# vitoplantamura/OnnxStream

Hardware: NVIDIA H100
Metric: SD1.5 UNet 512x512 bs=1 denoise steps/s (one UNet Model::run per step) (higher is better)
Workload: dtype f16

## Files before the change

### include/onnxstream_b200_kernels.h

```cpp
#ifndef ONNXSTREAM_B200_KERNELS_H
#define ONNXSTREAM_B200_KERNELS_H

#include <stddef.h>
#include <stdint.h>

#ifdef __cplusplus
extern "C" {
#endif

enum { OSB_NONE = 0, OSB_U8 = 1, OSB_F16 = 2, OSB_F32 = 3, OSB_I64 = 4 };

#define OSB_MAX_DIMS 6

int osb_convert(const void* src, int src_dtype, void* dst, int dst_dtype, size_t n, float scale, int zero_point, void* stream);

enum { OSB_UN_SIGMOID = 0, OSB_UN_SILU, OSB_UN_ERF, OSB_UN_SQRT, OSB_UN_SIN, OSB_UN_COS, OSB_UN_POW, OSB_UN_NEG,
       OSB_UN_GELU_ERF, OSB_UN_COPY, OSB_UN_MULC, OSB_UN_ADDC, OSB_UN_RECIP_SQRT };
int osb_unary(int op, const void* x, void* y, int dtype, size_t n, float alpha, void* stream);

enum { OSB_BIN_ADD = 0, OSB_BIN_SUB, OSB_BIN_MUL, OSB_BIN_DIV, OSB_BIN_MUL_GELU, OSB_BIN_MUL_SIGMOID, OSB_BIN_SILU_MUL  };
int osb_binary(int op, const void* a, const int64_t* a_strides, const void* b, const int64_t* b_strides,
               void* out, const int64_t* out_shape, int ndim, int dtype, void* stream);

int osb_bf16x3_expand_cols(const void* in_f32, void* out_bf16, int64_t rows, int64_t L, int64_t ld_in, int b_side, void* stream);
int osb_bf16x3_expand_rows(const void* in_f32, void* out_bf16, int64_t K, int64_t N, int b_side, void* stream);
int osb_tc_gemm_f32x_ok(int64_t M, int64_t N, int64_t K);
int osb_tc_conv_f32x_ok(int64_t H, int64_t W, int64_t Cin, int64_t Cout, int kh, int kw, int stride, int64_t Ho, int64_t Wo);
int osb_tc_gemm_f32x(const void* A6, const void* B6, void* C_f32, const void* bias_f32, const void* residual_f32, int64_t M, int64_t N, int64_t K6, int b_transposed, void* stream);
int osb_tc_conv_f32x(const void* x6, const void* w6, const void* bias_f32, const void* residual_f32, void* y_f32, int64_t H, int64_t W, int64_t Cin6, int64_t Cout,
                     int kh, int kw, int stride, int pad_top, int pad_left, int64_t Ho, int64_t Wo, void* stream);
int osb_concat2(const void* a, const void* b, void* out, int64_t outer, int64_t a_bytes, int64_t b_bytes, void* stream);
int osb_strided_copy(const void* in, void* out, int elem_size, int ndim, const int64_t* shape,
                     const int64_t* in_stride, const int64_t* in_div, int64_t in_offset,
                     const int64_t* out_stride, int64_t out_offset, void* stream);

int osb_transpose2d(const void* in, void* out, int elem_size, int64_t batch, int64_t rows, int64_t cols, void* stream);

int osb_softmax(const void* x, void* y, int dtype, int64_t rows, int64_t cols, void* stream);

int osb_softmax_scaled(const void* x, void* y, int dtype, int64_t rows, int64_t cols, float scale, const void* mask, int64_t mask_rows, void* stream);
int osb_softmax_scaled_ld(const void* x, void* y, int dtype, int64_t rows, int64_t cols, int64_t ld, float scale, const void* mask, int64_t mask_rows, void* stream);

int osb_instance_norm(const void* x, void* y, int dtype, int64_t channels, int64_t n_per_channel,
                      const void* scale, const void* bias, float eps, void* stream);

int osb_group_norm(const void* x, void* y, int dtype, int nhwc, int64_t C, int64_t HW, int groups,
                   const void* gamma, const void* beta, float eps, int fuse_silu, void* stats, void* stream);

int osb_geglu(const void* x, void* y, int dtype, int64_t rows, int64_t inner, void* stream);

int osb_layer_norm(const void* x, void* y, int dtype, int64_t rows, int64_t cols, const void* gamma, const void* beta,
                   float eps, void* stream);

int osb_reduce_mean(const void* x, void* y, int dtype, int64_t rows, int64_t cols, void* stream);

int osb_gather_rows(const void* table, const int64_t* idx, void* out, int64_t n_idx, int64_t table_rows, int64_t row_bytes, void* stream);

int osb_gemm(const void* A, const void* B, void* C, const void* bias, const void* residual,
             int64_t batch, int64_t M, int64_t N, int64_t K,
             int64_t stride_a, int64_t stride_b, int64_t stride_c, int b_transposed, int dtype, int impl, void* stream);

int osb_gemm_grouped(const void* A, const void* const* B, void* const* C, int groups, int64_t M, int64_t N, int64_t K,
                     int b_transposed, int dtype, int impl, void* stream);

int osb_gemm_ld(const void* A, int64_t lda, const void* B, int64_t ldb, void* C, int64_t ldc, const void* bias, const void* residual,
                int64_t batch, int64_t M, int64_t N, int64_t K, int64_t stride_a, int64_t stride_b, int64_t stride_c,
                int b_transposed, int dtype, int impl, void* stream);

int osb_conv2d(const void* x, const void* w, const void* bias, const void* residual, void* y,
               int64_t H, int64_t W, int64_t Cin, int64_t Cout, int kh, int kw, int stride, int pad_top, int pad_left,
               int64_t Ho, int64_t Wo, int dtype, int impl, void* stream);
int osb_conv2d_ex(const void* x, const void* w, const void* bias, const void* bias2, const void* residual, void* y, int64_t H, int64_t W, int64_t Cin, int64_t Cout,
                  int kh, int kw, int stride, int pad_top, int pad_left, int64_t Ho, int64_t Wo, int dtype, int impl, void* stream,
                  void* gn_stats, int gn_groups, int* gn_done);
int osb_conv2d_fusable(const void* x, const void* w, const void* y, int64_t H, int64_t W, int64_t Cin, int64_t Cout, int kh, int kw, int stride, int dtype, int impl);
int osb_rms_norm(const void* x, int xd, const void* w, int wd, void* y, int yd, int64_t rows, int64_t cols, float eps, void* stream);
int osb_rope(const void* x, const void* cs, const void* sn, void* y, int dtype, int64_t rows, int64_t D, int64_t table_rows, void* stream);
int osb_gemv_w8(const void* A, const void* Wq, void* C, const void* bias, const void* residual, int64_t M, int64_t N, int64_t K, float wscale, int wzp, int dtype, void* stream);
int osb_gemv_grouped(const void* A, const void* const* B, void* const* C, const int64_t* N, const float* wscale, const int* wzp, int groups,
                     int64_t M, int64_t K, int wdtype, int dtype, void* stream);
int osb_qu8_tc_gemm_ok(int64_t M, int64_t N, int64_t K, const void* A, const void* B, const void* C);
int osb_qu8_tc_conv_ok(int64_t Cin, int64_t Cout, int64_t Ho, int64_t Wo, int kh, int kw, int stride, const void* x, const void* w, const void* y);
int osb_rowsum_u8(const void* x, void* out, int64_t rows, int64_t cols, void* stream);
int osb_colsum_u8(const void* w, void* out, int64_t K, int64_t N, void* stream);
int osb_pad_sum_u8(const void* x, void* xp, void* psum, int64_t H, int64_t W, int64_t C, int64_t Hp, int64_t Wp, int pad_top, int pad_left, int zx, void* stream);
int osb_qu8_tc_gemm(const void* A, const void* B, void* C, const void* bias, const void* rsum, const void* csum, int64_t M, int64_t N, int64_t K, int bt,
                    int zx, float sx, int zw, float sw, int zy, float sy, void* stream);
int osb_qu8_tc_conv(const void* xp, const void* psum, const void* w, const void* bias, const void* csum, void* y, int64_t Hp, int64_t Wp, int64_t Cin, int64_t Cout,
                    int kh, int kw, int stride, int64_t Ho, int64_t Wo, int zx, float sx, int zw, float sw, int zy, float sy, void* stream);
int osb_binary_qu8(int op, const void* a, const int64_t* as, float sa, int za, const void* b, const int64_t* bs, float sb, int zb,
                   void* out, float so, int zo, const int64_t* shape, int ndim, void* stream);
int osb_softmax_qu8(const void* x, void* y, int64_t rows, int64_t cols, float in_scale, float out_scale, int out_zp, void* stream);
int osb_percentiles(const void* x, int dtype, size_t n, int threads, float from_left, float from_right, void* out3, void* stream);
float osb_percentile_key_to_float(unsigned key, int dtype);
int osb_channel_add_stats(const void* x, const void* addv, void* y, int dtype, int64_t C, int64_t HW, int groups, void* stats, void* stream);
int osb_group_norm_apply(const void* x, void* y, int dtype, int64_t C, int64_t HW, int groups, const void* gamma, const void* beta, float eps, int fuse_silu,
                         const void* stats, void* clear_stats, void* stream);

int osb_attention(const void* q, const void* k, const void* v, const void* mask, void* out,
                  int64_t heads, int64_t Tq, int64_t Tk, int64_t d, int64_t dv, float scale, int k_transposed,
                  int64_t kv_group, int dtype, void* stream);

int osb_flash_attention_ok(int64_t T, int64_t Tk, int64_t d, int dtype);
int osb_flash_attention(const void* q, int64_t ldq, const void* k, int64_t ldk, const void* v, int64_t ldv, void* out, int64_t ldo,
                        int64_t heads, int64_t T, int64_t Tk, int64_t d, float scale, void* stream);

int osb_flash_attention_f32x_ok(int64_t T, int64_t Tk, int64_t d, int dtype);
int osb_flash_attention_f32x(const void* q, int64_t ldq, const void* k, int64_t ldk, const void* v, int64_t ldv, void* out, int64_t ldo,
                             int64_t heads, int64_t T, int64_t Tk, int64_t d, float scale, void* planes, void* stream);

int osb_flash_attention_wide_ok(int64_t T, int64_t Tk, int64_t d, int dtype);
int osb_flash_attention_wide(const void* q, const void* k, const void* v, void* out, int64_t heads, int64_t T, int64_t Tk, int64_t d,
                             float scale, int k_transposed, int dtype, void* stream);

int osb_flash_attention_wide_f32x_ok(int64_t T, int64_t Tk, int64_t d, int dtype);
int osb_flash_attention_wide_f32x(const void* q, const void* k, const void* v, void* out, int64_t heads, int64_t T, int64_t Tk, int64_t d,
                                  float scale, int k_transposed, void* planes, void* stream);

int osb_sdpa_flash_ok(int64_t Hq, int64_t Hkv, int64_t Tq, int64_t Tk, int64_t d, int64_t dv, int dtype);
int osb_sdpa_flash(const void* q, const void* k, const void* v, const void* mask, void* out,
                   int64_t Hq, int64_t Hkv, int64_t Tq, int64_t Tk, int64_t d, float scale, void* stream);

int osb_gemm_qu8(const uint8_t* A, const uint8_t* B, uint8_t* C, const int32_t* bias, int64_t M, int64_t N, int64_t K,
                 int zx, float sx, int zw, float sw, int zy, float sy, void* stream);
int osb_conv2d_qu8(const uint8_t* x, const uint8_t* w, const int32_t* bias, uint8_t* y,
                   int64_t H, int64_t W, int64_t Cin, int64_t Cout, int kh, int kw, int stride, int pad_top, int pad_left,
                   int64_t Ho, int64_t Wo, int zx, float sx, int zw, float sw, int zy, float sy, void* stream);

int osb_scatter_elems(void* out, const int64_t* pos, const void* updates, int64_t n, int elem_size, void* stream);

int osb_maxpool_nhwc(const void* x, void* y, int dtype, int64_t H, int64_t W, int64_t C, int kh, int kw, int stride, int pad_top,
                     int pad_left, int64_t Ho, int64_t Wo, void* stream);

int osb_fill(void* dst, int dtype, size_t n, float value, void* stream);

int osb_gemm_tc_eligible(int64_t M, int64_t N, int64_t K, int dtype);

void osb_tc_set_pair_mode(int mode);

void osb_tc_profile(int enable);
int osb_tc_profile_read(double* out4);
int osb_tc_profile_dump(char* buf, int cap);

int osb_pdl_enabled(void);
void osb_set_pdl(int enable);

uint64_t osb_launch_count(void);
void osb_launch_count_reset(void);
uint64_t osb_tc_launch_count(void);

#ifdef __cplusplus
}
#endif
#endif
```

### onnxstream_b200/csrc/gemm_wgmma.cu

```cuda

#include "common.cuh"
#include "workspace.h"
#include "tc_ptx.cuh"
#include <cuda.h>
#include <cstdio>
#include <cstdlib>
#include <vector>

namespace {

constexpr int BLOCK_M = 128;
constexpr int BLOCK_N = 128;
constexpr int BLOCK_K = 64;
constexpr int WG_K = 16;
constexpr int STAGES = 6;
constexpr int A_STAGE_BYTES = BLOCK_M * BLOCK_K * 2;
constexpr int B_STAGE_BYTES = BLOCK_N * BLOCK_K * 2;
constexpr int SMEM_BYTES = STAGES * (A_STAGE_BYTES + B_STAGE_BYTES) + 1024  + 256  + 2 * tcptx::GN_MAX_GROUPS * 4;
constexpr int NUM_THREADS = 384;
constexpr int CONSUMER_THREADS = 256;

struct TcParams {
    int M, N, K;
    int batch;
    int m_tiles, n_tiles;
    int b_kmajor;
    int a_swap, b_swap;
    int taps, kw, pad_top, pad_left, Wo, Ho, bw, bh, tiles_x;
    int k_blocks_per_tap;
    int stride;
    int split_k;
    float* ws;
    int groups;
    __half* C1;
    __half* C2;
    __half* C;
    const __half* bias;
    const __half* bias2;
    const __half* residual;
    double* gn_stats;
    int gn_cpg, gn_groups;
    int gn_debug;
    int bf16;
    int f32_out;
    long long stride_c;
    long long ldc;
};

using namespace tcptx;

template <int B_MN_MAJOR, bool BF16>
__device__ __forceinline__ void mma_kblock(float (&acc)[64], uint64_t adesc, uint64_t bdesc)
{
    constexpr uint32_t b_kstep = B_MN_MAJOR ? (WG_K * 128) >> 4 : (WG_K * 2) >> 4;
    wgmma_fence();
#pragma unroll
    for (int k = 0; k < BLOCK_K / WG_K; k++) {
        const uint64_t a = adesc + (uint64_t)(k * ((WG_K * 2) >> 4)), b = bdesc + (uint64_t)(k * b_kstep);
        if (BF16) wgmma_m64n128k16_bf16<B_MN_MAJOR>(acc, a, b, 1u);
        else wgmma_m64n128k16_f16<B_MN_MAJOR>(acc, a, b, 1u);
    }
    wgmma_commit();
}


template <bool EXTRAS, int B_MN_MAJOR, bool BF16, bool PAIR>
__global__ void __launch_bounds__(NUM_THREADS, 1)
tc_gemm_kernel(const __grid_constant__ CUtensorMap map_a, const __grid_constant__ CUtensorMap map_b, const __grid_constant__ CUtensorMap map_b1,
               const __grid_constant__ CUtensorMap map_b2, const TcParams p)
{
    osb_pdl_trigger_entry();
    extern __shared__ uint8_t smem_raw[];
    uint8_t* smem = (uint8_t*)(((uintptr_t)smem_raw + 1023) & ~(uintptr_t)1023);
    uint8_t* smem_a = smem;
    uint8_t* smem_b = smem + STAGES * A_STAGE_BYTES;
    uint64_t* bars = (uint64_t*)(smem + STAGES * (A_STAGE_BYTES + B_STAGE_BYTES));
    uint64_t* full = bars;
    uint64_t* empty = bars + STAGES;
    float* gn_acc = (float*)((uint8_t*)bars + 256);

    const int warp = threadIdx.x >> 5;
    const int lane = threadIdx.x & 31;
    if (EXTRAS && p.gn_stats && threadIdx.x < 2 * GN_MAX_GROUPS) gn_acc[threadIdx.x] = 0.f;

    if (warp == 0 && lane == 0) {
        asm volatile("prefetch.tensormap [%0];" ::"l"(&map_a) : "memory");
        asm volatile("prefetch.tensormap [%0];" ::"l"(&map_b) : "memory");
    }
    constexpr uint32_t EMPTY_ARRIVALS = PAIR ? 2 * (CONSUMER_THREADS / 32) : CONSUMER_THREADS;
    if (warp == 1 && lane == 0) {
        for (int i = 0; i < STAGES; i++) { mbar_init(&full[i], 1); mbar_init(&empty[i], EMPTY_ARRIVALS); }
        asm volatile("fence.mbarrier_init.release.cluster;" ::: "memory");
    }
    if (PAIR) cluster_sync();
    else __syncthreads();
    osb_pdl_wait();

    const uint32_t rank = PAIR ? cluster_ctarank() : 0;
    const int first = PAIR ? (int)cluster_id_x() : (int)blockIdx.x, step = PAIR ? (int)cluster_count_x() : (int)gridDim.x;
    const int m_units = PAIR ? (p.m_tiles + 1) / 2 : p.m_tiles;
    const int tiles_per_batch = m_units * p.n_tiles;
    const int total_tiles = tiles_per_batch * p.batch * p.split_k;
    const int k_blocks_all = p.taps * p.k_blocks_per_tap;
    const int kb_per_split = (k_blocks_all + p.split_k - 1) / p.split_k;

    if (warp == 0) {
        const uint32_t sa0 = smem_u32(smem_a), sb0 = smem_u32(smem_b);
        int stage = 0; uint32_t phase = 0;
        for (int tile = first; tile < total_tiles; tile += step) {
            int sp = tile % p.split_k, t2 = tile / p.split_k;
            int b = t2 / tiles_per_batch, r = t2 % tiles_per_batch;
            int mt = r % m_units, nt = r / m_units;
            if (PAIR) mt = 2 * mt + (int)rank;
            int n0 = nt * BLOCK_N;
            int y0 = 0, x0 = 0, m0 = mt * BLOCK_M;
            if (p.taps > 1 || p.bh > 0) { y0 = (mt / p.tiles_x) * p.bh; x0 = (mt % p.tiles_x) * p.bw; }
            const CUtensorMap* mbp = &map_b;
            if (p.groups > 1) { if (b == 1) mbp = &map_b1; else if (b == 2) mbp = &map_b2; b = 0; }
            int kb_lo = sp * kb_per_split, kb_hi = min(kb_lo + kb_per_split, k_blocks_all);
            int tap = kb_lo / p.k_blocks_per_tap, kcb = kb_lo % p.k_blocks_per_tap;
            int ky = tap / p.kw, kx = tap % p.kw;
            const int ax = x0 * p.stride - p.pad_left, ay = y0 * p.stride - p.pad_top;
            for (int kb = kb_lo; kb < kb_hi; kb++) {
                mbar_wait(&empty[stage], phase ^ 1);
                if (elect_one()) {
                    mbar_expect_tx(&full[stage], A_STAGE_BYTES + B_STAGE_BYTES);
                    const int kc = kcb * BLOCK_K;
                    const uint32_t sa = sa0 + stage * A_STAGE_BYTES;
                    const uint32_t sb = sb0 + stage * B_STAGE_BYTES;
                    if (p.bh > 0) tma_load_3d_s(sa, &map_a, &full[stage], kc, ax + kx, ay + ky);
                    else if (p.a_swap) tma_load_3d_s(sa, &map_a, &full[stage], kc, b, m0);
                    else tma_load_3d_s(sa, &map_a, &full[stage], kc, m0, b);
                    const int kglob = tap * p.K + kc;
                    if (PAIR) {
                        const uint32_t sbh = sb + rank * (B_STAGE_BYTES / 2);
                        const int nh = n0 + 64 * (int)rank;
                        if (p.b_kmajor) {
                            if (p.b_swap) tma_load_3d_mc(sbh, mbp, &full[stage], kglob, b, nh, 0x3);
                            else tma_load_3d_mc(sbh, mbp, &full[stage], kglob, nh, b, 0x3);
                        } else {
                            if (p.b_swap) tma_load_3d_mc(sbh, mbp, &full[stage], nh, b, kglob, 0x3);
                            else tma_load_3d_mc(sbh, mbp, &full[stage], nh, kglob, b, 0x3);
                        }
                    } else if (p.b_kmajor) {
                        if (p.b_swap) tma_load_3d_s(sb, mbp, &full[stage], kglob, b, n0);
                        else tma_load_3d_s(sb, mbp, &full[stage], kglob, n0, b);
                    } else {
                        if (p.b_swap) {
                            tma_load_3d_s(sb, mbp, &full[stage], n0, b, kglob);
                            tma_load_3d_s(sb + B_STAGE_BYTES / 2, mbp, &full[stage], n0 + 64, b, kglob);
                        } else {
                            tma_load_3d_s(sb, mbp, &full[stage], n0, kglob, b);
                            tma_load_3d_s(sb + B_STAGE_BYTES / 2, mbp, &full[stage], n0 + 64, kglob, b);
                        }
                    }
                }
                __syncwarp();
                if (++kcb == p.k_blocks_per_tap) { kcb = 0; tap++; if (++kx == p.kw) { kx = 0; ky++; } }
                if (++stage == STAGES) { stage = 0; phase ^= 1; }
            }
        }
        osb_pdl_trigger_late();
    } else if (warp >= 4) {
        const int wg = (warp >> 2) - 1;
        const int ct = (int)threadIdx.x - (NUM_THREADS - CONSUMER_THREADS);
        const uint64_t adesc0 = make_smem_desc(smem_u32(smem_a) + wg * (BLOCK_M / 2) * 128, 16, 1024);
        const uint64_t bdesc0 = p.b_kmajor ? make_smem_desc(smem_u32(smem_b), 16, 1024) : make_smem_desc(smem_u32(smem_b), B_STAGE_BYTES / 2, 1024);
        const bool partial = p.split_k > 1 || p.f32_out;
        const int r_lo = wg * 64 + (warp & 3) * 16 + (lane >> 2);
        const int cq = 2 * (lane & 3);
        auto release = [&](int s) {
            if (PAIR) {
                __syncwarp();
                if (lane == 0) { mbar_arrive(&empty[s]); mbar_arrive_remote(&empty[s], rank ^ 1u); }
            } else {
                mbar_arrive(&empty[s]);
            }
        };
        int stage = 0; uint32_t phase = 0;
        for (int tile = first; tile < total_tiles; tile += step) {
            int sp = tile % p.split_k, t2 = tile / p.split_k;
            int b = t2 / tiles_per_batch, r = t2 % tiles_per_batch;
            int mt = r % m_units, nt = r / m_units;
            if (PAIR) mt = 2 * mt + (int)rank;
            const int n0 = nt * BLOCK_N;
            const int n_end = min(p.N, n0 + BLOCK_N);
            const int kb_lo = sp * kb_per_split, kb_hi = min(kb_lo + kb_per_split, k_blocks_all);

            float acc[64];
#pragma unroll
            for (int i = 0; i < 64; i++) acc[i] = 0.f;
            int prev = -1;
            for (int kb = kb_lo; kb < kb_hi; kb++) {
                mbar_wait(&full[stage], phase);
                mma_kblock<B_MN_MAJOR, BF16>(acc, adesc0 + (uint64_t)(stage * (A_STAGE_BYTES >> 4)), bdesc0 + (uint64_t)(stage * (B_STAGE_BYTES >> 4)));
                if (prev >= 0) { wgmma_wait<1>(); release(prev); }
                prev = stage;
                if (++stage == STAGES) { stage = 0; phase ^= 1; }
            }
            wgmma_wait<0>();
            release(prev);

            long long out_row[2];
            bool row_ok[2];
#pragma unroll
            for (int h = 0; h < 2; h++) {
                const int row_in_tile = r_lo + 8 * h;
                if (p.bh > 0) {
                    int y = (mt / p.tiles_x) * p.bh + row_in_tile / p.bw, x = (mt % p.tiles_x) * p.bw + row_in_tile % p.bw;
                    row_ok[h] = y < p.Ho && x < p.Wo;
                    out_row[h] = (long long)y * p.Wo + x;
                } else {
                    int m = mt * BLOCK_M + row_in_tile;
                    row_ok[h] = m < p.M;
                    out_row[h] = m;
                }
            }
            __half* cbase = p.C;
            if (p.groups > 1) cbase = b == 0 ? p.C : (b == 1 ? p.C1 : p.C2);
            const bool pair_ok = (p.N & 1) == 0 && (p.ldc & 1) == 0;
#pragma unroll
            for (int j = 0; j < BLOCK_N / 8; j++) {
                if (n0 + 8 * j >= n_end) break;
                const int n = n0 + 8 * j + cq;
                const bool ok0 = n < n_end, ok1 = n + 1 < n_end;
                float s0 = 0.f, s1 = 0.f, q0 = 0.f, q1 = 0.f;
                float add0 = 0.f, add1 = 0.f;
                if (!partial) {
                    if (p.bias) { if (ok0) add0 += __half2float(p.bias[n]); if (ok1) add1 += __half2float(p.bias[n + 1]); }
                }
#pragma unroll
                for (int h = 0; h < 2; h++) {
                    if (!row_ok[h]) continue;
                    float f0 = acc[4 * j + 2 * h], f1 = acc[4 * j + 2 * h + 1];
                    if (partial) {
                        float* wrow = p.ws + (((long long)sp * p.batch + b) * p.M + out_row[h]) * p.N;
                        if (ok1 && pair_ok) *reinterpret_cast<float2*>(wrow + n) = make_float2(f0, f1);
                        else { if (ok0) wrow[n] = f0; if (ok1) wrow[n + 1] = f1; }
                        continue;
                    }
                    const long long off = (long long)b * p.stride_c + out_row[h] * p.ldc;
                    f0 += add0; f1 += add1;
                    if (p.residual) { if (ok0) f0 += __half2float(p.residual[off + n]); if (ok1) f1 += __half2float(p.residual[off + n + 1]); }
                    if (EXTRAS && p.bias2) { if (ok0) f0 += __half2float(p.bias2[n]); if (ok1) f1 += __half2float(p.bias2[n + 1]); }
                    const __half o0 = __float2half_rn(f0), o1 = __float2half_rn(f1);
                    __half* crow = cbase + off;
                    if (ok1 && pair_ok) *reinterpret_cast<__half2*>(crow + n) = __halves2half2(o0, o1);
                    else { if (ok0) crow[n] = o0; if (ok1) crow[n + 1] = o1; }
                    if (EXTRAS) {
                        const float g0 = ok0 ? __half2float(o0) : 0.f, g1 = ok1 ? __half2float(o1) : 0.f;
                        s0 += g0; q0 = fmaf(g0, g0, q0); s1 += g1; q1 = fmaf(g1, g1, q1);
                    }
                }
                if (EXTRAS && p.gn_stats && !partial && !(p.gn_debug & 1)) gn_stats_pair(s0, s1, q0, q1, n, n_end, p.gn_cpg, gn_acc, lane);
            }
            if (EXTRAS && p.gn_stats && !partial && !(p.gn_debug & 2)) {
                asm volatile("bar.sync 1, %0;" ::"n"(CONSUMER_THREADS) : "memory");
                gn_stats_flush(gn_acc, p.gn_stats, p.gn_groups, ct);
            }
        }
    }
    if (PAIR) cluster_sync();
}

__global__ void splitk_reduce_kernel(const float* __restrict__ ws, __half* __restrict__ out, const __half* __restrict__ bias, const __half* __restrict__ bias2,
                                     const __half* __restrict__ residual, long long rows, int N, int splits, double* __restrict__ gn_stats, int gn_cpg, int gn_groups)
{
    osb_pdl_prologue();
    __shared__ float acc[2 * GN_MAX_GROUPS];
    if (gn_stats) { if (threadIdx.x < 2 * GN_MAX_GROUPS) acc[threadIdx.x] = 0.f; __syncthreads(); }
    const long long total4 = rows * N / 4;
    const long long plane4 = total4;
    const float4* w4 = reinterpret_cast<const float4*>(ws);
    for (long long i = blockIdx.x * (long long)blockDim.x + threadIdx.x; i < total4; i += (long long)gridDim.x * blockDim.x) {
        float4 a = w4[i];
        for (int s = 1; s < splits; s++) { float4 t = w4[(long long)s * plane4 + i]; a.x += t.x; a.y += t.y; a.z += t.z; a.w += t.w; }
        long long e = i * 4;
        int n = (int)(e % N);
        if (bias) { a.x += __half2float(bias[n]); a.y += __half2float(bias[n + 1]); a.z += __half2float(bias[n + 2]); a.w += __half2float(bias[n + 3]); }
        if (bias2) { a.x += __half2float(bias2[n]); a.y += __half2float(bias2[n + 1]); a.z += __half2float(bias2[n + 2]); a.w += __half2float(bias2[n + 3]); }
        if (residual) {
            Vec<__half, 4> r = load_vec<__half, 4>(residual + e);
            a.x += __half2float(r.v[0]); a.y += __half2float(r.v[1]); a.z += __half2float(r.v[2]); a.w += __half2float(r.v[3]);
        }
        Vec<__half, 4> o;
        o.v[0] = __float2half_rn(a.x); o.v[1] = __float2half_rn(a.y); o.v[2] = __float2half_rn(a.z); o.v[3] = __float2half_rn(a.w);
        store_vec<__half, 4>(out + e, o);
        if (gn_stats) {
            float x0 = __half2float(o.v[0]), x1 = __half2float(o.v[1]), x2 = __half2float(o.v[2]), x3 = __half2float(o.v[3]);
            const int g = n / gn_cpg;
            atomicAdd(&acc[2 * g], (x0 + x1) + (x2 + x3));
            atomicAdd(&acc[2 * g + 1], fmaf(x0, x0, x1 * x1) + fmaf(x2, x2, x3 * x3));
        }
    }
    if (gn_stats) {
        __syncthreads();
        if (threadIdx.x < 2 * gn_groups) { float v = acc[threadIdx.x]; if (v != 0.f) atomicAdd(&gn_stats[threadIdx.x], (double)v); }
    }
}

__global__ void splitk_reduce_f32_kernel(const float* __restrict__ ws, float* __restrict__ out, const float* __restrict__ bias, const float* __restrict__ residual,
                                         long long rows, int N, int splits)
{
    osb_pdl_prologue();
    const long long total = rows * N;
    for (long long i = blockIdx.x * (long long)blockDim.x + threadIdx.x; i < total; i += (long long)gridDim.x * blockDim.x) {
        float a = ws[i];
        for (int s = 1; s < splits; s++) a += ws[(long long)s * total + i];
        if (bias) a += bias[(int)(i % N)];
        if (residual) a += residual[i];
        out[i] = a;
    }
}

#include "gemm_i8.cuh"

constexpr size_t WS_MAX = OSB_WS_SPLITK_BYTES;

int num_sms();

int choose_split(int tiles, int k_blocks, size_t out_elems, cudaStream_t st, OsbWorkspace** ws_out)
{
    static const int forced = [] { const char* e = getenv("OSB_TC_SPLIT"); return e ? atoi(e) : 0; }();
    *ws_out = nullptr;
    static const int min_kb = [] { const char* e = getenv("OSB_TC_SPLIT_MINKB"); int v = e ? atoi(e) : 0; return v > 0 ? v : 32; }();
    if ((tiles >= 100 && forced <= 0) || k_blocks < 4 || (k_blocks < min_kb && forced <= 0)) return 1;
    int split = forced > 0 ? forced : num_sms() / tiles;
    split = std::min(split, k_blocks / 2);
    while (split > 1 && (size_t)split * out_elems * 4 > WS_MAX) split--;
    if (split <= 1) return 1;
    int kb_per = (k_blocks + split - 1) / split;
    split = (k_blocks + kb_per - 1) / kb_per;
    if (split <= 1) return 1;
    OsbWorkspace* ws = osb_workspace(st, OSB_WS_SPLITK);
    if (!ws) return 1;
    *ws_out = ws;
    return split;
}

bool make_map_rb(CUtensorMap* map, const void* base, uint64_t inner, uint64_t rows, uint64_t batch, uint64_t row_stride_bytes, uint64_t batch_stride_bytes,
                 uint32_t box_inner, uint32_t box_rows, int* swapped)
{
    if (batch > 1 && batch_stride_bytes < row_stride_bytes) {
        *swapped = 1;
        return make_map(map, base, inner, batch, rows, batch_stride_bytes, row_stride_bytes, box_inner, 1, box_rows);
    }
    *swapped = 0;
    return make_map(map, base, inner, rows, batch, row_stride_bytes, batch_stride_bytes, box_inner, box_rows, 1);
}

int num_sms()
{
    static int n = 0;
    if (!n) { int dev = 0; cudaGetDevice(&dev); cudaDeviceGetAttribute(&n, cudaDevAttrMultiProcessorCount, dev); if (n <= 0) n = 132; }
    return n;
}

struct ProfRec { cudaEvent_t a, b; double flops, bytes; int M, N, K, taps, batch, split, conv; };
bool g_prof = false;
std::vector<ProfRec> g_prof_list;

void prof_begin(ProfRec& rec, const TcParams& p, cudaStream_t st)
{
    cudaEventCreate(&rec.a); cudaEventCreate(&rec.b);
    const double kdiv = p.bf16 ? 6.0 : 1.0, es = p.bf16 ? 4.0 : 2.0;
    double M = p.M, N = p.N, Kt = (double)p.K * p.taps / kdiv, B = p.batch;
    rec.flops = 2.0 * M * N * Kt * B;
    double a_bytes = (p.bh > 0 ? M * (p.K / kdiv) : M * Kt) * es * B;
    rec.bytes = a_bytes + N * Kt * es * (p.bh > 0 ? 1.0 : B) + M * N * es * B * (p.residual ? 2.0 : 1.0) + (p.bias ? N * es : 0.0);
    rec.M = p.M; rec.N = p.N; rec.K = p.K; rec.taps = p.taps; rec.batch = p.batch; rec.split = p.split_k; rec.conv = p.bh > 0;
    cudaEventRecord(rec.a, st);
}

using TcKernel = void (*)(CUtensorMap, CUtensorMap, CUtensorMap, CUtensorMap, TcParams);

int launch(const CUtensorMap& ma, const CUtensorMap& mb, const TcParams& p, cudaStream_t st, const CUtensorMap* mb1p = nullptr, const CUtensorMap* mb2p = nullptr,
           bool pair = false)
{
    const CUtensorMap& mb1 = mb1p ? *mb1p : mb;
    const CUtensorMap& mb2 = mb2p ? *mb2p : mb;
    static bool attr_set = false;
    if (!attr_set) {
        TcKernel kernels[] = {
            tc_gemm_kernel<false, 0, false, false>, tc_gemm_kernel<false, 1, false, false>, tc_gemm_kernel<true, 0, false, false>, tc_gemm_kernel<true, 1, false, false>,
            tc_gemm_kernel<false, 0, true, false>, tc_gemm_kernel<false, 1, true, false>,
            tc_gemm_kernel<false, 0, false, true>, tc_gemm_kernel<false, 1, false, true>, tc_gemm_kernel<true, 0, false, true>, tc_gemm_kernel<true, 1, false, true> };
        for (auto k : kernels) {
            cudaError_t e = cudaFuncSetAttribute(k, cudaFuncAttributeMaxDynamicSharedMemorySize, SMEM_BYTES);
            if (e != cudaSuccess) return (int)e;
        }
        attr_set = true;
    }
    const bool extras = p.bias2 != nullptr || p.gn_stats != nullptr;
    TcKernel k;
    if (pair) {
        if (p.bf16 || p.split_k != 1 || p.groups > 1) return (int)cudaErrorInvalidValue;
        k = extras ? (p.b_kmajor ? tc_gemm_kernel<true, 0, false, true> : tc_gemm_kernel<true, 1, false, true>)
                   : (p.b_kmajor ? tc_gemm_kernel<false, 0, false, true> : tc_gemm_kernel<false, 1, false, true>);
    } else if (p.bf16) {
        k = p.b_kmajor ? tc_gemm_kernel<false, 0, true, false> : tc_gemm_kernel<false, 1, true, false>;
    } else if (extras) {
        k = p.b_kmajor ? tc_gemm_kernel<true, 0, false, false> : tc_gemm_kernel<true, 1, false, false>;
    } else {
        k = p.b_kmajor ? tc_gemm_kernel<false, 0, false, false> : tc_gemm_kernel<false, 1, false, false>;
    }
    int grid;
    if (pair) {
        static int max_clusters = 0;
        if (!max_clusters) {
            cudaLaunchConfig_t cfg{};
            cfg.gridDim = dim3(2 * (num_sms() / 2)); cfg.blockDim = dim3(NUM_THREADS); cfg.dynamicSmemBytes = SMEM_BYTES;
            cudaLaunchAttribute attr[1];
            attr[0].id = cudaLaunchAttributeClusterDimension;
            attr[0].val.clusterDim.x = 2; attr[0].val.clusterDim.y = 1; attr[0].val.clusterDim.z = 1;
            cfg.attrs = attr; cfg.numAttrs = 1;
            int n = 0;
            if (cudaOccupancyMaxActiveClusters(&n, k, &cfg) != cudaSuccess || n <= 0) { cudaGetLastError(); n = num_sms() / 2; }
            max_clusters = std::min(n, num_sms() / 2);
        }
        const int units = (p.m_tiles + 1) / 2 * p.n_tiles * p.batch;
        grid = 2 * std::min(units, max_clusters);
    } else {
        grid = std::min(p.m_tiles * p.n_tiles * p.batch * p.split_k, num_sms());
    }
    ProfRec rec{};
    if (g_prof) prof_begin(rec, p, st);
    osb_launch_cluster(k, grid, NUM_THREADS, (size_t)SMEM_BYTES, st, pair ? 2u : 1u, ma, mb, mb1, mb2, p);
    if (p.f32_out) {
        launched(1);
        const long long total = (long long)p.batch * p.M * p.N;
        int rgrid = (int)std::min<long long>((total + 255) / 256, num_sms() * 8);
        osb_launch((splitk_reduce_f32_kernel), rgrid, 256, 0, st, (const float*)p.ws, (float*)p.C, (const float*)p.bias, (const float*)p.residual, (long long)p.batch * p.M, p.N, p.split_k);
        if (g_prof) { cudaEventRecord(rec.b, st); g_prof_list.push_back(rec); }
        return launched(0);
    }
    if (p.split_k > 1) {
        launched(1);
        long long total4 = (long long)p.batch * p.M * p.N / 4;
        int rgrid = (int)std::min<long long>((total4 + 255) / 256, num_sms() * 8);
        osb_launch((splitk_reduce_kernel), rgrid, 256, 0, st, (const float*)p.ws, p.C, p.bias, p.bias2, p.residual, (long long)p.batch * p.M, p.N, p.split_k,
                   p.gn_stats, p.gn_cpg, p.gn_groups);
        if (g_prof) { cudaEventRecord(rec.b, st); g_prof_list.push_back(rec); }
        return launched(0);
    }
    if (g_prof) { cudaEventRecord(rec.b, st); g_prof_list.push_back(rec); }
    return launched(1);
}

int env_int(const char* name)
{
    const char* e = getenv(name);
    return e ? atoi(e) : 0;
}

inline uint32_t next_pow2(uint32_t v) { uint32_t r = 1; while (r < v) r <<= 1; return r; }

int g_pair_mode = -1;
int pair_mode()
{
    if (g_pair_mode < 0) { const char* e = getenv("OSB_TC_PAIR"); g_pair_mode = e ? atoi(e) : 1; }
    return g_pair_mode;
}

bool use_pair(int64_t m_tiles, int64_t N)
{
    return pair_mode() == 2 && m_tiles >= 2 && N % 8 == 0;
}

}

extern "C" void osb_tc_set_pair_mode(int mode) { g_pair_mode = mode; }

extern "C" void osb_tc_profile(int enable)
{
    for (auto& r : g_prof_list) { cudaEventDestroy(r.a); cudaEventDestroy(r.b); }
    g_prof_list.clear();
    g_prof = enable != 0;
}

extern "C" int osb_tc_profile_read(double* out4)
{
    double ms = 0, fl = 0, by = 0;
    for (auto& r : g_prof_list) {
        if (cudaEventSynchronize(r.b) != cudaSuccess) return -1;
        float t = 0.f;
        if (cudaEventElapsedTime(&t, r.a, r.b) != cudaSuccess) return -1;
        ms += t; fl += r.flops; by += r.bytes;
    }
    out4[0] = (double)g_prof_list.size(); out4[1] = ms; out4[2] = fl; out4[3] = by;
    return 0;
}

extern "C" int osb_tc_profile_dump(char* buf, int cap)
{
    int off = 0;
    for (auto& r : g_prof_list) {
        float t = 0.f;
        if (cudaEventSynchronize(r.b) != cudaSuccess || cudaEventElapsedTime(&t, r.a, r.b) != cudaSuccess) return -1;
        int n = snprintf(buf + off, cap - off, "%d %d %d %d %d %d %d %.4f %.3f\n", r.M, r.N, r.K, r.taps, r.batch, r.split, r.conv, t, r.flops * 1e-9);
        if (n < 0 || off + n >= cap) break;
        off += n;
    }
    return off;
}


extern "C" int osb_qu8_tc_gemm_ok(int64_t M, int64_t N, int64_t K, const void* A, const void* B, const void* C)
{
    if (M < 32 || N < 16 || K < 16 || (N % 16) || (K % 16)) return 0;
    if (((uintptr_t)A | (uintptr_t)B | (uintptr_t)C) & 15) return 0;
    static const int off = env_int("OSB_QU8_TC_OFF");
    return get_encode() != nullptr && !off;
}

extern "C" int osb_qu8_tc_conv_ok(int64_t Cin, int64_t Cout, int64_t Ho, int64_t Wo, int kh, int kw, int stride, const void* x, const void* w, const void* y)
{
    if ((Cin % 16) || (Cout % 16) || Ho * Wo < 64 || kh > 7 || kw > 7 || stride < 1 || stride > 2) return 0;
    if (((uintptr_t)x | (uintptr_t)w | (uintptr_t)y) & 15) return 0;
    static const int off = env_int("OSB_QU8_TC_OFF");
    return get_encode() != nullptr && !off;
}

extern "C" int osb_rowsum_u8(const void* x, void* out, int64_t rows, int64_t cols, void* stream)
{
    if (rows * cols == 0) return 0;
    osb_launch((i8k::rowsum_u8_kernel), (unsigned)std::min<int64_t>((rows + 7) / 8, num_sms() * 8), 256, 0, (cudaStream_t)stream, (const uint8_t*)x, (int32_t*)out, (long long)rows, (long long)cols);
    return launched();
}

extern "C" int osb_colsum_u8(const void* w, void* out, int64_t K, int64_t N, void* stream)
{
    if (K * N == 0) return 0;
    cudaStream_t st = (cudaStream_t)stream;
    cudaError_t e = cudaMemsetAsync(out, 0, (size_t)N * 4, st);
    if (e != cudaSuccess) return (int)e;
    const int64_t gx = (N + 255) / 256;
    const int64_t gy = std::max<int64_t>(1, std::min<int64_t>((K + 63) / 64, (num_sms() * 4 + gx - 1) / gx));
    const int64_t k_per = (K + gy - 1) / gy;
    osb_launch((i8k::colsum_u8_kernel), dim3((unsigned)gx, (unsigned)((K + k_per - 1) / k_per)), 256, 0, st, (const uint8_t*)w, (int32_t*)out, (long long)K, (long long)N, (long long)k_per);
    return launched();
}

extern "C" int osb_pad_sum_u8(const void* x, void* xp, void* psum, int64_t H, int64_t W, int64_t C, int64_t Hp, int64_t Wp, int pad_top, int pad_left, int zx, void* stream)
{
    if (Hp * Wp * C == 0) return 0;
    if (C % 16) return (int)cudaErrorInvalidValue;
    osb_launch((i8k::pad_sum_u8_kernel), (unsigned)std::min<int64_t>((Hp * Wp + 7) / 8, num_sms() * 16), 256, 0, (cudaStream_t)stream, (const uint8_t*)x, (uint8_t*)xp, (int32_t*)psum,
               (int)H, (int)W, (int)C, (int)Hp, (int)Wp, pad_top, pad_left, zx);
    return launched();
}

static int launch_i8(const CUtensorMap& ma, const CUtensorMap& mb, const i8k::I8Params& p, cudaStream_t st)
{
    static bool attr_set = false;
    if (!attr_set) {
        cudaError_t e = cudaFuncSetAttribute(i8k::tc_i8_kernel, cudaFuncAttributeMaxDynamicSharedMemorySize, i8k::I8_SMEM);
        if (e != cudaSuccess) return (int)e;
        attr_set = true;
    }
    const int total = p.m_tiles * p.n_tiles;
    osb_launch((i8k::tc_i8_kernel), std::min(total, num_sms()), NUM_THREADS, (size_t)i8k::I8_SMEM, st, ma, mb, p);
    return launched(1);
}

extern "C" int osb_qu8_tc_gemm(const void* A, const void* B, void* C, const void* bias, const void* rsum, const void* csum, int64_t M, int64_t N, int64_t K, int bt,
                               int zx, float sx, int zw, float sw, int zy, float sy, void* stream)
{
    CUtensorMap ma, mb;
    if (!make_map(&ma, A, (uint64_t)K, (uint64_t)M, 1, (uint64_t)K, (uint64_t)M * K, i8k::I8_BLOCK_K, BLOCK_M, 1, 1, CU_TENSOR_MAP_DATA_TYPE_UINT8)) return (int)cudaErrorInvalidValue;
    bool ok = bt ? make_map(&mb, B, (uint64_t)K, (uint64_t)N, 1, (uint64_t)K, (uint64_t)N * K, i8k::I8_BLOCK_K, BLOCK_N, 1, 1, CU_TENSOR_MAP_DATA_TYPE_UINT8)
                 : make_map(&mb, B, (uint64_t)N, (uint64_t)K, 1, (uint64_t)N, (uint64_t)N * K, BLOCK_N, i8k::I8_BLOCK_K, 1, 1, CU_TENSOR_MAP_DATA_TYPE_UINT8);
    if (!ok) return (int)cudaErrorInvalidValue;
    i8k::I8Params p{};
    p.M = (int)M; p.N = (int)N; p.K = (int)K;
    p.m_tiles = (int)((M + BLOCK_M - 1) / BLOCK_M); p.n_tiles = (int)((N + BLOCK_N - 1) / BLOCK_N);
    p.b_kmajor = bt ? 1 : 0;
    p.taps = 1; p.kw = 1; p.bh = 0; p.bw = 0; p.tiles_x = 1; p.stride = 1;
    p.k_blocks_per_tap = (int)((K + i8k::I8_BLOCK_K - 1) / i8k::I8_BLOCK_K);
    p.rsum = (const int32_t*)rsum; p.csum = (const int32_t*)csum; p.bias = (const int32_t*)bias;
    p.zx = zx; p.zw = zw; p.zy = zy; p.kzz = (int)(K * zx * zw); p.requant = sx * sw / sy;
    p.C = (uint8_t*)C; p.ldc = N;
    return launch_i8(ma, mb, p, (cudaStream_t)stream);
}

extern "C" int osb_qu8_tc_conv(const void* xp, const void* psum, const void* w, const void* bias, const void* csum, void* y, int64_t Hp, int64_t Wp, int64_t Cin, int64_t Cout,
                               int kh, int kw, int stride, int64_t Ho, int64_t Wo, int zx, float sx, int zw, float sw, int zy, float sy, void* stream)
{
    const uint32_t bw = std::min<uint32_t>(128, next_pow2((uint32_t)Wo)), bh = 128 / bw;
    CUtensorMap ma, mb;
    const int64_t Ktot = (int64_t)kh * kw * Cin;
    if (!make_map(&ma, xp, (uint64_t)Cin, (uint64_t)Wp, (uint64_t)Hp, (uint64_t)Cin, (uint64_t)Wp * Cin, i8k::I8_BLOCK_K, bw * stride, bh * stride, (uint32_t)stride, CU_TENSOR_MAP_DATA_TYPE_UINT8))
        return (int)cudaErrorInvalidValue;
    if (!make_map(&mb, w, (uint64_t)Ktot, (uint64_t)Cout, 1, (uint64_t)Ktot, (uint64_t)Ktot * Cout, i8k::I8_BLOCK_K, BLOCK_N, 1, 1, CU_TENSOR_MAP_DATA_TYPE_UINT8)) return (int)cudaErrorInvalidValue;
    i8k::I8Params p{};
    p.M = (int)(Ho * Wo); p.N = (int)Cout; p.K = (int)Cin;
    p.tiles_x = (int)((Wo + bw - 1) / bw);
    p.m_tiles = p.tiles_x * (int)((Ho + bh - 1) / bh);
    p.n_tiles = (int)((Cout + BLOCK_N - 1) / BLOCK_N);
    p.b_kmajor = 1;
    p.taps = kh * kw; p.kw = kw; p.Wo = (int)Wo; p.Ho = (int)Ho; p.bw = (int)bw; p.bh = (int)bh; p.stride = stride; p.Wp = (int)Wp;
    p.k_blocks_per_tap = (int)((Cin + i8k::I8_BLOCK_K - 1) / i8k::I8_BLOCK_K);
    p.rsum = (const int32_t*)psum; p.csum = (const int32_t*)csum; p.bias = (const int32_t*)bias;
    p.zx = zx; p.zw = zw; p.zy = zy; p.kzz = (int)(Ktot * zx * zw); p.requant = sx * sw / sy;
    p.C = (uint8_t*)y; p.ldc = Cout;
    return launch_i8(ma, mb, p, (cudaStream_t)stream);
}

bool osb_tc_gemm_ok(int64_t M, int64_t N, int64_t K, int bt, const void* A, const void* B, const void* C, int64_t sa, int64_t sb, int64_t sc,
                    int64_t lda, int64_t ldb, int64_t ldc)
{
    if ((lda % 8) || (ldb % 8) || (ldc % 8)) return false;
    if (M < 32 || N < 1 || K < 8) return false;
    if (K % 8) return false;
    if (N % 8) return false;
    if (M > (1 << 30) || N > (1 << 30) || K > (1 << 30)) return false;
    if (((uintptr_t)A | (uintptr_t)B | (uintptr_t)C) & 15) return false;
    if ((sa % 8) || (sb % 8) || (sc % 8)) return false;
    (void)bt;
    return get_encode() != nullptr || A == nullptr;
}

static thread_local int g_f32x = 0;

static bool f32x_params(TcParams& p, OsbWorkspace* wsp, cudaStream_t st)
{
    p.bf16 = 1; p.f32_out = 1;
    p.bias2 = nullptr; p.gn_stats = nullptr;
    if ((size_t)p.split_k * p.batch * p.M * p.N * 4 > WS_MAX) p.split_k = 1;
    if ((size_t)p.batch * p.M * p.N * 4 > WS_MAX) return false;
    if (!wsp) wsp = osb_workspace(st, OSB_WS_SPLITK);
    if (!wsp) return false;
    p.ws = wsp->splitk;
    return true;
}

int osb_tc_gemm_launch(const void* A, const void* B, void* C, const void* bias, const void* residual, int64_t batch, int64_t M, int64_t N, int64_t K,
                       int64_t sa, int64_t sb, int64_t sc, int bt, cudaStream_t st, int64_t lda, int64_t ldb, int64_t ldc)
{
    if (g_f32x && batch != 1) return (int)cudaErrorNotSupported;
    if (lda <= 0) lda = K;
    if (ldb <= 0) ldb = bt ? K : N;
    if (ldc <= 0) ldc = N;
    CUtensorMap ma, mb;
    uint64_t abatch = sa ? (uint64_t)batch : 1, bbatch = sb ? (uint64_t)batch : 1;
    if (batch > 1 && (!sa || !sb)) {
        for (int64_t i = 0; i < batch; i++) {
            int r = osb_tc_gemm_launch((const __half*)A + i * sa, (const __half*)B + i * sb, (__half*)C + i * sc, bias,
                                       residual ? (const __half*)residual + i * sc : nullptr, 1, M, N, K, M * lda, bt ? N * ldb : K * ldb, sc, bt, st, lda, ldb, ldc);
            if (r) return r;
        }
        return 0;
    }
    int a_swap = 0, b_swap = 0;
    if (!make_map_rb(&ma, A, (uint64_t)K, (uint64_t)M, abatch, (uint64_t)lda * 2, (uint64_t)(sa ? sa : M * lda) * 2, BLOCK_K, BLOCK_M, &a_swap)) return (int)cudaErrorInvalidValue;
    int64_t m_tiles = (M + BLOCK_M - 1) / BLOCK_M;
    const bool pair = !g_f32x && use_pair(m_tiles, N);
    bool okb = bt ? make_map_rb(&mb, B, (uint64_t)K, (uint64_t)N, bbatch, (uint64_t)ldb * 2, (uint64_t)(sb ? sb : N * ldb) * 2, BLOCK_K, pair ? BLOCK_N / 2 : BLOCK_N, &b_swap)
                  : make_map_rb(&mb, B, (uint64_t)N, (uint64_t)K, bbatch, (uint64_t)ldb * 2, (uint64_t)(sb ? sb : K * ldb) * 2, 64, BLOCK_K, &b_swap);
    if (!okb) return (int)cudaErrorInvalidValue;
    TcParams p{};
    p.M = (int)M; p.N = (int)N; p.K = (int)K; p.batch = (int)batch;
    p.m_tiles = (int)m_tiles; p.n_tiles = (int)((N + BLOCK_N - 1) / BLOCK_N);
    p.b_kmajor = bt ? 1 : 0;
    p.a_swap = a_swap; p.b_swap = b_swap;
    p.taps = 1; p.kw = 1; p.bh = 0; p.bw = 0; p.tiles_x = 1;
    p.k_blocks_per_tap = (int)((K + BLOCK_K - 1) / BLOCK_K);
    p.stride = 1;
    p.C = (__half*)C; p.bias = (const __half*)bias; p.residual = (const __half*)residual; p.stride_c = sc; p.ldc = ldc;
    if (pair) { p.split_k = 1; return launch(ma, mb, p, st, nullptr, nullptr, true); }
    OsbWorkspace* wsp = nullptr;
    const bool split_ok = ldc == N && (sc == M * N || batch == 1) && ((uintptr_t)residual & 7) == 0;
    p.split_k = split_ok ? choose_split(p.m_tiles * p.n_tiles * p.batch, p.k_blocks_per_tap, (size_t)batch * M * N, st, &wsp) : 1;
    p.ws = wsp ? wsp->splitk : nullptr;
    if (g_f32x && !f32x_params(p, wsp, st)) return (int)cudaErrorNotSupported;
    return launch(ma, mb, p, st);
}

int osb_tc_gemm_grouped_launch(const void* A, const void* const* B, void* const* C, int groups, int64_t M, int64_t N, int64_t K, int bt, cudaStream_t st,
                               int64_t lda, int64_t ldb, int64_t ldc)
{
    if (groups < 2 || groups > 3) return (int)cudaErrorInvalidValue;
    CUtensorMap ma, mb[3];
    int a_swap = 0, b_swap = 0;
    if (!make_map_rb(&ma, A, (uint64_t)K, (uint64_t)M, 1, (uint64_t)lda * 2, (uint64_t)(M * lda) * 2, BLOCK_K, BLOCK_M, &a_swap)) return (int)cudaErrorInvalidValue;
    int64_t m_tiles = (M + BLOCK_M - 1) / BLOCK_M;
    for (int g = 0; g < groups; g++) {
        int sw = 0;
        bool ok = bt ? make_map_rb(&mb[g], B[g], (uint64_t)K, (uint64_t)N, 1, (uint64_t)ldb * 2, (uint64_t)(N * ldb) * 2, BLOCK_K, BLOCK_N, &sw)
                     : make_map_rb(&mb[g], B[g], (uint64_t)N, (uint64_t)K, 1, (uint64_t)ldb * 2, (uint64_t)(K * ldb) * 2, 64, BLOCK_K, &sw);
        if (!ok || (g > 0 && sw != b_swap)) return (int)cudaErrorInvalidValue;
        b_swap = sw;
    }
    TcParams p{};
    p.M = (int)M; p.N = (int)N; p.K = (int)K; p.batch = groups; p.groups = groups;
    p.m_tiles = (int)m_tiles; p.n_tiles = (int)((N + BLOCK_N - 1) / BLOCK_N);
    p.b_kmajor = bt ? 1 : 0;
    p.a_swap = a_swap; p.b_swap = b_swap;
    p.taps = 1; p.kw = 1; p.bh = 0; p.bw = 0; p.tiles_x = 1;
    p.k_blocks_per_tap = (int)((K + BLOCK_K - 1) / BLOCK_K);
    p.stride = 1;
    p.C = (__half*)C[0]; p.C1 = (__half*)C[1]; p.C2 = (__half*)(groups > 2 ? C[2] : C[1]);
    p.bias = nullptr; p.residual = nullptr; p.stride_c = 0; p.ldc = ldc;
    p.split_k = 1; p.ws = nullptr;
    return launch(ma, mb[0], p, st, &mb[1], groups > 2 ? &mb[2] : &mb[1]);
}

bool osb_tc_conv_ok(int64_t H, int64_t W, int64_t Cin, int64_t Cout, int kh, int kw, int stride, const void* x, const void* w, const void* y)
{
    if (stride < 1 || stride > 2) return false;
    if (Cin % 8 || Cin < 16) return false;
    if (H * W < 64) return false;
    if (kh > 7 || kw > 7) return false;
    if (((uintptr_t)x | (uintptr_t)w | (uintptr_t)y) & 15) return false;
    return get_encode() != nullptr;
}

int osb_tc_conv_launch(const void* x, const void* w, const void* bias, const void* residual, void* y, int64_t H, int64_t W, int64_t Cin, int64_t Cout,
                       int kh, int kw, int stride, int pad_top, int pad_left, int64_t Ho, int64_t Wo, cudaStream_t st,
                       const void* bias2, double* gn_stats, int gn_groups, int* gn_done)
{
    if (gn_done) *gn_done = 0;
    if (gn_stats && (gn_groups < 1 || gn_groups > tcptx::GN_MAX_GROUPS || Cout % gn_groups || Cout % 8)) gn_stats = nullptr;
    const int gn_cpg = gn_stats ? (int)(Cout / gn_groups) : 0;
    uint32_t bw = std::min<uint32_t>(128, next_pow2((uint32_t)Wo)), bh = 128 / bw;
    CUtensorMap ma, mb;
    if (!make_map(&ma, x, (uint64_t)Cin, (uint64_t)W, (uint64_t)H, (uint64_t)Cin * 2, (uint64_t)W * Cin * 2, BLOCK_K, bw * stride, bh * stride, (uint32_t)stride))
        return (int)cudaErrorInvalidValue;
    int64_t Ktot = (int64_t)kh * kw * Cin;
    const int64_t m_tiles_ = ((Wo + bw - 1) / bw) * ((Ho + bh - 1) / bh);
    const bool pair = !g_f32x && Cout % 8 == 0 && use_pair(m_tiles_, Cout);
    if (!make_map(&mb, w, (uint64_t)Ktot, (uint64_t)Cout, 1, (uint64_t)Ktot * 2, (uint64_t)Ktot * Cout * 2, BLOCK_K, pair ? BLOCK_N / 2 : BLOCK_N, 1))
        return (int)cudaErrorInvalidValue;
    TcParams p{};
    p.M = (int)(Ho * Wo); p.N = (int)Cout; p.K = (int)Cin; p.batch = 1;
    p.tiles_x = (int)((Wo + bw - 1) / bw);
    p.m_tiles = p.tiles_x * (int)((Ho + bh - 1) / bh);
    p.n_tiles = (int)((Cout + BLOCK_N - 1) / BLOCK_N);
    p.b_kmajor = 1;
    p.taps = kh * kw; p.kw = kw; p.pad_top = pad_top; p.pad_left = pad_left; p.Wo = (int)Wo; p.Ho = (int)Ho; p.bw = (int)bw; p.bh = (int)bh;
    p.k_blocks_per_tap = (int)((Cin + BLOCK_K - 1) / BLOCK_K);
    p.stride = stride;
    p.C = (__half*)y; p.bias = (const __half*)bias; p.residual = (const __half*)residual; p.stride_c = 0; p.ldc = Cout;
    if (pair) {
        p.split_k = 1;
        p.bias2 = (const __half*)bias2;
        if (gn_stats) { p.gn_stats = gn_stats; p.gn_cpg = gn_cpg; p.gn_groups = gn_groups; if (gn_done) *gn_done = 1; }
        { static const int dbg = env_int("OSB_GN_DEBUG"); p.gn_debug = dbg; }
        return launch(ma, mb, p, st, nullptr, nullptr, true);
    }
    OsbWorkspace* wsp = nullptr;
    p.split_k = (Cout % 4 == 0 && ((uintptr_t)residual & 7) == 0) ? choose_split(p.m_tiles * p.n_tiles, p.taps * p.k_blocks_per_tap, (size_t)Ho * Wo * Cout, st, &wsp) : 1;
    p.ws = wsp ? wsp->splitk : nullptr;
    p.bias2 = (const __half*)bias2;
    const bool stats_ok = gn_stats && (p.split_k == 1 || gn_cpg % 4 == 0);
    if (stats_ok) { p.gn_stats = gn_stats; p.gn_cpg = gn_cpg; p.gn_groups = gn_groups; if (gn_done) *gn_done = 1; }
    { static const int dbg = env_int("OSB_GN_DEBUG"); p.gn_debug = dbg; }
    if (g_f32x) {
        if (!f32x_params(p, wsp, st)) return (int)cudaErrorNotSupported;
    }
    return launch(ma, mb, p, st);
}

extern "C" int osb_tc_gemm_f32x_ok(int64_t M, int64_t N, int64_t K)
{
    static const bool on = [] { const char* e = getenv("OSB_F32_TC"); return !(e && e[0] == '0'); }();
    return on && M >= 32 && N >= 8 && N % 8 == 0 && K >= 8 && (6 * K) % 8 == 0 && (size_t)M * N * 4 <= WS_MAX && get_encode() != nullptr ? 1 : 0;
}
extern "C" int osb_tc_conv_f32x_ok(int64_t H, int64_t W, int64_t Cin, int64_t Cout, int kh, int kw, int stride, int64_t Ho, int64_t Wo)
{
    static const bool on = [] { const char* e = getenv("OSB_F32_TC"); return !(e && e[0] == '0'); }();
    return on && (6 * Cin) % 8 == 0 && 6 * Cin >= 16 && stride >= 1 && stride <= 2 && H * W >= 64 && kh <= 7 && kw <= 7 && (size_t)Ho * Wo * Cout * 4 <= WS_MAX &&
           get_encode() != nullptr ? 1 : 0;
}

extern "C" int osb_tc_gemm_f32x(const void* A6, const void* B6, void* C, const void* bias, const void* residual, int64_t M, int64_t N, int64_t K6, int bt, void* stream)
{
    const int64_t ldb = bt ? K6 : N;
    if (!osb_tc_gemm_ok(M, N, K6, bt, A6, B6, nullptr, 0, 0, 0, K6, ldb, 8) || (N % 8)) return (int)cudaErrorNotSupported;
    g_f32x = 1;
    int r = osb_tc_gemm_launch(A6, B6, C, bias, residual, 1, M, N, K6, 0, 0, M * N, bt, (cudaStream_t)stream, K6, ldb, N);
    g_f32x = 0;
    return r;
}

extern "C" int osb_tc_conv_f32x(const void* x6, const void* w6, const void* bias, const void* residual, void* y, int64_t H, int64_t W, int64_t Cin6, int64_t Cout,
                     int kh, int kw, int stride, int pad_top, int pad_left, int64_t Ho, int64_t Wo, void* stream)
{
    if (!osb_tc_conv_ok(H, W, Cin6, Cout, kh, kw, stride, x6, w6, nullptr)) return (int)cudaErrorNotSupported;
    g_f32x = 1;
    int r = osb_tc_conv_launch(x6, w6, bias, residual, y, H, W, Cin6, Cout, kh, kw, stride, pad_top, pad_left, Ho, Wo, (cudaStream_t)stream, nullptr, nullptr, 0, nullptr);
    g_f32x = 0;
    return r;
}
```

### onnxstream_b200/csrc/tc_ptx.cuh

```cuda
#pragma once
#include "common.cuh"
#include <cuda.h>
#include <cudaTypedefs.h>
#include <cstdio>
#include <mutex>

namespace tcptx {


inline PFN_cuTensorMapEncodeTiled_v12000 get_encode()
{
    static PFN_cuTensorMapEncodeTiled_v12000 fn = nullptr;
    static std::once_flag once;
    std::call_once(once, [] {
        void* p = nullptr;
        cudaDriverEntryPointQueryResult q;
        if (cudaGetDriverEntryPoint("cuTensorMapEncodeTiled", &p, cudaEnableDefault, &q) == cudaSuccess && q == cudaDriverEntryPointSuccess)
            fn = (PFN_cuTensorMapEncodeTiled_v12000)p;
    });
    return fn;
}

inline bool make_map(CUtensorMap* map, const void* base, uint64_t d0, uint64_t d1, uint64_t d2, uint64_t s1_bytes, uint64_t s2_bytes,
                     uint32_t b0, uint32_t b1, uint32_t b2, uint32_t traversal_stride = 1, CUtensorMapDataType dtype = CU_TENSOR_MAP_DATA_TYPE_FLOAT16)
{
    auto enc = get_encode();
    if (!enc) return false;
    cuuint64_t dims[3] = { d0, d1, d2 };
    cuuint64_t strides[2] = { s1_bytes, s2_bytes };
    cuuint32_t box[3] = { b0, b1, b2 };
    cuuint32_t estr[3] = { 1, traversal_stride, traversal_stride };
    CUresult r = enc(map, dtype, 3, const_cast<void*>(base), dims, strides, box, estr,
                     CU_TENSOR_MAP_INTERLEAVE_NONE, CU_TENSOR_MAP_SWIZZLE_128B, CU_TENSOR_MAP_L2_PROMOTION_L2_256B,
                     CU_TENSOR_MAP_FLOAT_OOB_FILL_NONE);
    return r == CUDA_SUCCESS;
}


__device__ __forceinline__ uint32_t smem_u32(const void* p) { return (uint32_t)__cvta_generic_to_shared(p); }

__device__ __forceinline__ void mbar_init(uint64_t* bar, uint32_t count)
{
    asm volatile("mbarrier.init.shared::cta.b64 [%0], %1;" ::"r"(smem_u32(bar)), "r"(count));
}
__device__ __forceinline__ void mbar_expect_tx(uint64_t* bar, uint32_t bytes)
{
    asm volatile("mbarrier.arrive.expect_tx.shared::cta.b64 _, [%0], %1;" ::"r"(smem_u32(bar)), "r"(bytes) : "memory");
}
__device__ __forceinline__ void mbar_arrive(uint64_t* bar)
{
    asm volatile("mbarrier.arrive.shared::cta.b64 _, [%0];" ::"r"(smem_u32(bar)) : "memory");
}
__device__ __forceinline__ void mbar_wait(uint64_t* bar, uint32_t parity)
{
    uint32_t addr = smem_u32(bar);
    uint32_t done = 0;
    long long t0 = 0;
    while (true) {
        asm volatile(
            "{\n\t"
            ".reg .pred p;\n\t"
            "mbarrier.try_wait.parity.shared::cta.b64 p, [%1], %2;\n\t"
            "selp.u32 %0, 1, 0, p;\n\t"
            "}" : "=r"(done) : "r"(addr), "r"(parity) : "memory");
        if (done) break;
        long long now = clock64();
        if (t0 == 0) t0 = now;
        else if (now - t0 > 4000000000LL) __trap();
    }
}

__device__ __forceinline__ void tma_load_3d(void* smem, const CUtensorMap* map, uint64_t* bar, int c0, int c1, int c2)
{
    asm volatile("cp.async.bulk.tensor.3d.shared::cluster.global.mbarrier::complete_tx::bytes [%0], [%1, {%3, %4, %5}], [%2];"
                 ::"r"(smem_u32(smem)), "l"(map), "r"(smem_u32(bar)), "r"(c0), "r"(c1), "r"(c2) : "memory");
}
__device__ __forceinline__ void tma_load_3d_s(uint32_t smem_addr, const CUtensorMap* map, uint64_t* bar, int c0, int c1, int c2)
{
    asm volatile("cp.async.bulk.tensor.3d.shared::cluster.global.mbarrier::complete_tx::bytes [%0], [%1, {%3, %4, %5}], [%2];"
                 ::"r"(smem_addr), "l"(map), "r"(smem_u32(bar)), "r"(c0), "r"(c1), "r"(c2) : "memory");
}
__device__ __forceinline__ void tma_load_3d_mc(uint32_t smem_addr, const CUtensorMap* map, uint64_t* bar, int c0, int c1, int c2, uint16_t cta_mask)
{
    asm volatile("cp.async.bulk.tensor.3d.shared::cluster.global.mbarrier::complete_tx::bytes.multicast::cluster [%0], [%1, {%3, %4, %5}], [%2], %6;"
                 ::"r"(smem_addr), "l"(map), "r"(smem_u32(bar)), "r"(c0), "r"(c1), "r"(c2), "h"(cta_mask) : "memory");
}

__device__ __forceinline__ uint32_t cluster_ctarank() { uint32_t r; asm volatile("mov.u32 %0, %%cluster_ctarank;" : "=r"(r)); return r; }
__device__ __forceinline__ uint32_t cluster_id_x() { uint32_t r; asm volatile("mov.u32 %0, %%clusterid.x;" : "=r"(r)); return r; }
__device__ __forceinline__ uint32_t cluster_count_x() { uint32_t r; asm volatile("mov.u32 %0, %%nclusterid.x;" : "=r"(r)); return r; }
__device__ __forceinline__ void cluster_sync()
{
    asm volatile("barrier.cluster.arrive.release;\n\tbarrier.cluster.wait.acquire;" ::: "memory");
}
__device__ __forceinline__ void mbar_arrive_remote(uint64_t* bar, uint32_t cta)
{
    asm volatile("{\n\t.reg .b32 ra;\n\tmapa.shared::cluster.u32 ra, %0, %1;\n\tmbarrier.arrive.release.cluster.shared::cluster.b64 _, [ra];\n\t}"
                 ::"r"(smem_u32(bar)), "r"(cta) : "memory");
}

__device__ __forceinline__ bool elect_one()
{
    uint32_t pred = 0;
    asm volatile("{\n\t.reg .pred px;\n\telect.sync _|px, 0xffffffff;\n\tselp.u32 %0, 1, 0, px;\n\t}" : "=r"(pred));
    return pred != 0;
}

__device__ __forceinline__ void named_bar_sync(uint32_t id, uint32_t count) { asm volatile("bar.sync %0, %1;" ::"r"(id), "r"(count) : "memory"); }
__device__ __forceinline__ void named_bar_arrive(uint32_t id, uint32_t count) { asm volatile("bar.arrive %0, %1;" ::"r"(id), "r"(count) : "memory"); }

template <int N>
__device__ __forceinline__ void setmaxnreg_dec() { asm volatile("setmaxnreg.dec.sync.aligned.u32 %0;" ::"n"(N)); }
template <int N>
__device__ __forceinline__ void setmaxnreg_inc() { asm volatile("setmaxnreg.inc.sync.aligned.u32 %0;" ::"n"(N)); }

template <int N>
__device__ __forceinline__ void fence_regs(float (&r)[N])
{
#pragma unroll
    for (int i = 0; i < N; i++) asm volatile("" : "+f"(r[i])::"memory");
}
template <int N>
__device__ __forceinline__ void fence_regs(uint32_t (&r)[N][4])
{
#pragma unroll
    for (int i = 0; i < N; i++)
#pragma unroll
        for (int e = 0; e < 4; e++) asm volatile("" : "+r"(r[i][e])::"memory");
}

__device__ __forceinline__ uint64_t make_smem_desc(uint32_t smem_addr, uint32_t lbo_bytes, uint32_t sbo_bytes)
{
    uint64_t d = 0;
    d |= (uint64_t)((smem_addr >> 4) & 0x3FFF);
    d |= (uint64_t)((lbo_bytes >> 4) & 0x3FFF) << 16;
    d |= (uint64_t)((sbo_bytes >> 4) & 0x3FFF) << 32;
    d |= (uint64_t)1 << 62;
    return d;
}

__device__ __forceinline__ void wgmma_fence() { asm volatile("wgmma.fence.sync.aligned;" ::: "memory"); }
__device__ __forceinline__ void wgmma_commit() { asm volatile("wgmma.commit_group.sync.aligned;" ::: "memory"); }
template <int N>
__device__ __forceinline__ void wgmma_wait() { asm volatile("wgmma.wait_group.sync.aligned %0;" ::"n"(N) : "memory"); }

template <int TRANS_B>
__device__ __forceinline__ void wgmma_m64n128k16_f16(float (&d)[64], uint64_t da, uint64_t db, uint32_t scale_d)
{
    asm volatile(
        "{\n\t.reg .pred p;\n\tsetp.ne.b32 p, %66, 0;\n\t"
        "wgmma.mma_async.sync.aligned.m64n128k16.f32.f16.f16 "
        "{%0, %1, %2, %3, %4, %5, %6, %7, %8, %9, %10, %11, %12, %13, %14, %15, %16, %17, %18, %19, %20, %21, %22, %23, %24, %25, %26, %27, %28, %29, %30, %31, %32, %33, %34, %35, %36, %37, %38, %39, %40, %41, %42, %43, %44, %45, %46, %47, %48, %49, %50, %51, %52, %53, %54, %55, %56, %57, %58, %59, %60, %61, %62, %63}, %64, %65, p, 1, 1, 0, %67;\n\t}"
        : "+f"(d[0]), "+f"(d[1]), "+f"(d[2]), "+f"(d[3]), "+f"(d[4]), "+f"(d[5]), "+f"(d[6]), "+f"(d[7]), "+f"(d[8]), "+f"(d[9]), "+f"(d[10]), "+f"(d[11]), "+f"(d[12]), "+f"(d[13]), "+f"(d[14]), "+f"(d[15]), "+f"(d[16]), "+f"(d[17]), "+f"(d[18]), "+f"(d[19]), "+f"(d[20]), "+f"(d[21]), "+f"(d[22]), "+f"(d[23]), "+f"(d[24]), "+f"(d[25]), "+f"(d[26]), "+f"(d[27]), "+f"(d[28]), "+f"(d[29]), "+f"(d[30]), "+f"(d[31]), "+f"(d[32]), "+f"(d[33]), "+f"(d[34]), "+f"(d[35]), "+f"(d[36]), "+f"(d[37]), "+f"(d[38]), "+f"(d[39]), "+f"(d[40]), "+f"(d[41]), "+f"(d[42]), "+f"(d[43]), "+f"(d[44]), "+f"(d[45]), "+f"(d[46]), "+f"(d[47]), "+f"(d[48]), "+f"(d[49]), "+f"(d[50]), "+f"(d[51]), "+f"(d[52]), "+f"(d[53]), "+f"(d[54]), "+f"(d[55]), "+f"(d[56]), "+f"(d[57]), "+f"(d[58]), "+f"(d[59]), "+f"(d[60]), "+f"(d[61]), "+f"(d[62]), "+f"(d[63])
        : "l"(da), "l"(db), "r"(scale_d), "n"(TRANS_B));
}
template <int TRANS_B>
__device__ __forceinline__ void wgmma_m64n64k16_f16(float (&d)[32], uint64_t da, uint64_t db, uint32_t scale_d)
{
    asm volatile(
        "{\n\t.reg .pred p;\n\tsetp.ne.b32 p, %34, 0;\n\t"
        "wgmma.mma_async.sync.aligned.m64n64k16.f32.f16.f16 "
        "{%0, %1, %2, %3, %4, %5, %6, %7, %8, %9, %10, %11, %12, %13, %14, %15, %16, %17, %18, %19, %20, %21, %22, %23, %24, %25, %26, %27, %28, %29, %30, %31}, %32, %33, p, 1, 1, 0, %35;\n\t}"
        : "+f"(d[0]), "+f"(d[1]), "+f"(d[2]), "+f"(d[3]), "+f"(d[4]), "+f"(d[5]), "+f"(d[6]), "+f"(d[7]), "+f"(d[8]), "+f"(d[9]), "+f"(d[10]), "+f"(d[11]), "+f"(d[12]), "+f"(d[13]), "+f"(d[14]), "+f"(d[15]), "+f"(d[16]), "+f"(d[17]), "+f"(d[18]), "+f"(d[19]), "+f"(d[20]), "+f"(d[21]), "+f"(d[22]), "+f"(d[23]), "+f"(d[24]), "+f"(d[25]), "+f"(d[26]), "+f"(d[27]), "+f"(d[28]), "+f"(d[29]), "+f"(d[30]), "+f"(d[31])
        : "l"(da), "l"(db), "r"(scale_d), "n"(TRANS_B));
}
template <int TRANS_B>
__device__ __forceinline__ void wgmma_m64n32k16_f16(float (&d)[16], uint64_t da, uint64_t db, uint32_t scale_d)
{
    asm volatile(
        "{\n\t.reg .pred p;\n\tsetp.ne.b32 p, %18, 0;\n\t"
        "wgmma.mma_async.sync.aligned.m64n32k16.f32.f16.f16 "
        "{%0, %1, %2, %3, %4, %5, %6, %7, %8, %9, %10, %11, %12, %13, %14, %15}, %16, %17, p, 1, 1, 0, %19;\n\t}"
        : "+f"(d[0]), "+f"(d[1]), "+f"(d[2]), "+f"(d[3]), "+f"(d[4]), "+f"(d[5]), "+f"(d[6]), "+f"(d[7]), "+f"(d[8]), "+f"(d[9]), "+f"(d[10]), "+f"(d[11]), "+f"(d[12]), "+f"(d[13]), "+f"(d[14]), "+f"(d[15])
        : "l"(da), "l"(db), "r"(scale_d), "n"(TRANS_B));
}
template <int TRANS_B>
__device__ __forceinline__ void wgmma_m64n128k16_bf16(float (&d)[64], uint64_t da, uint64_t db, uint32_t scale_d)
{
    asm volatile(
        "{\n\t.reg .pred p;\n\tsetp.ne.b32 p, %66, 0;\n\t"
        "wgmma.mma_async.sync.aligned.m64n128k16.f32.bf16.bf16 "
        "{%0, %1, %2, %3, %4, %5, %6, %7, %8, %9, %10, %11, %12, %13, %14, %15, %16, %17, %18, %19, %20, %21, %22, %23, %24, %25, %26, %27, %28, %29, %30, %31, %32, %33, %34, %35, %36, %37, %38, %39, %40, %41, %42, %43, %44, %45, %46, %47, %48, %49, %50, %51, %52, %53, %54, %55, %56, %57, %58, %59, %60, %61, %62, %63}, %64, %65, p, 1, 1, 0, %67;\n\t}"
        : "+f"(d[0]), "+f"(d[1]), "+f"(d[2]), "+f"(d[3]), "+f"(d[4]), "+f"(d[5]), "+f"(d[6]), "+f"(d[7]), "+f"(d[8]), "+f"(d[9]), "+f"(d[10]), "+f"(d[11]), "+f"(d[12]), "+f"(d[13]), "+f"(d[14]), "+f"(d[15]), "+f"(d[16]), "+f"(d[17]), "+f"(d[18]), "+f"(d[19]), "+f"(d[20]), "+f"(d[21]), "+f"(d[22]), "+f"(d[23]), "+f"(d[24]), "+f"(d[25]), "+f"(d[26]), "+f"(d[27]), "+f"(d[28]), "+f"(d[29]), "+f"(d[30]), "+f"(d[31]), "+f"(d[32]), "+f"(d[33]), "+f"(d[34]), "+f"(d[35]), "+f"(d[36]), "+f"(d[37]), "+f"(d[38]), "+f"(d[39]), "+f"(d[40]), "+f"(d[41]), "+f"(d[42]), "+f"(d[43]), "+f"(d[44]), "+f"(d[45]), "+f"(d[46]), "+f"(d[47]), "+f"(d[48]), "+f"(d[49]), "+f"(d[50]), "+f"(d[51]), "+f"(d[52]), "+f"(d[53]), "+f"(d[54]), "+f"(d[55]), "+f"(d[56]), "+f"(d[57]), "+f"(d[58]), "+f"(d[59]), "+f"(d[60]), "+f"(d[61]), "+f"(d[62]), "+f"(d[63])
        : "l"(da), "l"(db), "r"(scale_d), "n"(TRANS_B));
}
template <int TRANS_B>
__device__ __forceinline__ void wgmma_m64n64k16_bf16(float (&d)[32], uint64_t da, uint64_t db, uint32_t scale_d)
{
    asm volatile(
        "{\n\t.reg .pred p;\n\tsetp.ne.b32 p, %34, 0;\n\t"
        "wgmma.mma_async.sync.aligned.m64n64k16.f32.bf16.bf16 "
        "{%0, %1, %2, %3, %4, %5, %6, %7, %8, %9, %10, %11, %12, %13, %14, %15, %16, %17, %18, %19, %20, %21, %22, %23, %24, %25, %26, %27, %28, %29, %30, %31}, %32, %33, p, 1, 1, 0, %35;\n\t}"
        : "+f"(d[0]), "+f"(d[1]), "+f"(d[2]), "+f"(d[3]), "+f"(d[4]), "+f"(d[5]), "+f"(d[6]), "+f"(d[7]), "+f"(d[8]), "+f"(d[9]), "+f"(d[10]), "+f"(d[11]), "+f"(d[12]), "+f"(d[13]), "+f"(d[14]), "+f"(d[15]), "+f"(d[16]), "+f"(d[17]), "+f"(d[18]), "+f"(d[19]), "+f"(d[20]), "+f"(d[21]), "+f"(d[22]), "+f"(d[23]), "+f"(d[24]), "+f"(d[25]), "+f"(d[26]), "+f"(d[27]), "+f"(d[28]), "+f"(d[29]), "+f"(d[30]), "+f"(d[31])
        : "l"(da), "l"(db), "r"(scale_d), "n"(TRANS_B));
}
template <int TRANS_B>
__device__ __forceinline__ void wgmma_m64n32k16_bf16(float (&d)[16], uint64_t da, uint64_t db, uint32_t scale_d)
{
    asm volatile(
        "{\n\t.reg .pred p;\n\tsetp.ne.b32 p, %18, 0;\n\t"
        "wgmma.mma_async.sync.aligned.m64n32k16.f32.bf16.bf16 "
        "{%0, %1, %2, %3, %4, %5, %6, %7, %8, %9, %10, %11, %12, %13, %14, %15}, %16, %17, p, 1, 1, 0, %19;\n\t}"
        : "+f"(d[0]), "+f"(d[1]), "+f"(d[2]), "+f"(d[3]), "+f"(d[4]), "+f"(d[5]), "+f"(d[6]), "+f"(d[7]), "+f"(d[8]), "+f"(d[9]), "+f"(d[10]), "+f"(d[11]), "+f"(d[12]), "+f"(d[13]), "+f"(d[14]), "+f"(d[15])
        : "l"(da), "l"(db), "r"(scale_d), "n"(TRANS_B));
}
__device__ __forceinline__ void wgmma_m64n128k32_u8(int32_t (&d)[64], uint64_t da, uint64_t db, uint32_t scale_d)
{
    asm volatile(
        "{\n\t.reg .pred p;\n\tsetp.ne.b32 p, %66, 0;\n\t"
        "wgmma.mma_async.sync.aligned.m64n128k32.s32.u8.u8 "
        "{%0, %1, %2, %3, %4, %5, %6, %7, %8, %9, %10, %11, %12, %13, %14, %15, %16, %17, %18, %19, %20, %21, %22, %23, %24, %25, %26, %27, %28, %29, %30, %31, %32, %33, %34, %35, %36, %37, %38, %39, %40, %41, %42, %43, %44, %45, %46, %47, %48, %49, %50, %51, %52, %53, %54, %55, %56, %57, %58, %59, %60, %61, %62, %63}, %64, %65, p;\n\t}"
        : "+r"(d[0]), "+r"(d[1]), "+r"(d[2]), "+r"(d[3]), "+r"(d[4]), "+r"(d[5]), "+r"(d[6]), "+r"(d[7]), "+r"(d[8]), "+r"(d[9]), "+r"(d[10]), "+r"(d[11]), "+r"(d[12]), "+r"(d[13]), "+r"(d[14]), "+r"(d[15]), "+r"(d[16]), "+r"(d[17]), "+r"(d[18]), "+r"(d[19]), "+r"(d[20]), "+r"(d[21]), "+r"(d[22]), "+r"(d[23]), "+r"(d[24]), "+r"(d[25]), "+r"(d[26]), "+r"(d[27]), "+r"(d[28]), "+r"(d[29]), "+r"(d[30]), "+r"(d[31]), "+r"(d[32]), "+r"(d[33]), "+r"(d[34]), "+r"(d[35]), "+r"(d[36]), "+r"(d[37]), "+r"(d[38]), "+r"(d[39]), "+r"(d[40]), "+r"(d[41]), "+r"(d[42]), "+r"(d[43]), "+r"(d[44]), "+r"(d[45]), "+r"(d[46]), "+r"(d[47]), "+r"(d[48]), "+r"(d[49]), "+r"(d[50]), "+r"(d[51]), "+r"(d[52]), "+r"(d[53]), "+r"(d[54]), "+r"(d[55]), "+r"(d[56]), "+r"(d[57]), "+r"(d[58]), "+r"(d[59]), "+r"(d[60]), "+r"(d[61]), "+r"(d[62]), "+r"(d[63])
        : "l"(da), "l"(db), "r"(scale_d));
}
__device__ __forceinline__ void wgmma_m64n64k16_f16_rs(float (&d)[32], const uint32_t (&a)[4], uint64_t db, uint32_t scale_d)
{
    asm volatile(
        "{\n\t.reg .pred p;\n\tsetp.ne.b32 p, %37, 0;\n\t"
        "wgmma.mma_async.sync.aligned.m64n64k16.f32.f16.f16 "
        "{%0, %1, %2, %3, %4, %5, %6, %7, %8, %9, %10, %11, %12, %13, %14, %15, %16, %17, %18, %19, %20, %21, %22, %23, %24, %25, %26, %27, %28, %29, %30, %31}, {%32, %33, %34, %35}, %36, p, 1, 1, 1;\n\t}"
        : "+f"(d[0]), "+f"(d[1]), "+f"(d[2]), "+f"(d[3]), "+f"(d[4]), "+f"(d[5]), "+f"(d[6]), "+f"(d[7]), "+f"(d[8]), "+f"(d[9]), "+f"(d[10]), "+f"(d[11]), "+f"(d[12]), "+f"(d[13]), "+f"(d[14]), "+f"(d[15]), "+f"(d[16]), "+f"(d[17]), "+f"(d[18]), "+f"(d[19]), "+f"(d[20]), "+f"(d[21]), "+f"(d[22]), "+f"(d[23]), "+f"(d[24]), "+f"(d[25]), "+f"(d[26]), "+f"(d[27]), "+f"(d[28]), "+f"(d[29]), "+f"(d[30]), "+f"(d[31])
        : "r"(a[0]), "r"(a[1]), "r"(a[2]), "r"(a[3]), "l"(db), "r"(scale_d));
}
__device__ __forceinline__ void wgmma_m64n64k16_bf16_rs(float (&d)[32], const uint32_t (&a)[4], uint64_t db, uint32_t scale_d)
{
    asm volatile(
        "{\n\t.reg .pred p;\n\tsetp.ne.b32 p, %37, 0;\n\t"
        "wgmma.mma_async.sync.aligned.m64n64k16.f32.bf16.bf16 "
        "{%0, %1, %2, %3, %4, %5, %6, %7, %8, %9, %10, %11, %12, %13, %14, %15, %16, %17, %18, %19, %20, %21, %22, %23, %24, %25, %26, %27, %28, %29, %30, %31}, {%32, %33, %34, %35}, %36, p, 1, 1, 1;\n\t}"
        : "+f"(d[0]), "+f"(d[1]), "+f"(d[2]), "+f"(d[3]), "+f"(d[4]), "+f"(d[5]), "+f"(d[6]), "+f"(d[7]), "+f"(d[8]), "+f"(d[9]), "+f"(d[10]), "+f"(d[11]), "+f"(d[12]), "+f"(d[13]), "+f"(d[14]), "+f"(d[15]), "+f"(d[16]), "+f"(d[17]), "+f"(d[18]), "+f"(d[19]), "+f"(d[20]), "+f"(d[21]), "+f"(d[22]), "+f"(d[23]), "+f"(d[24]), "+f"(d[25]), "+f"(d[26]), "+f"(d[27]), "+f"(d[28]), "+f"(d[29]), "+f"(d[30]), "+f"(d[31])
        : "r"(a[0]), "r"(a[1]), "r"(a[2]), "r"(a[3]), "l"(db), "r"(scale_d));
}


constexpr int GN_MAX_GROUPS = 64;

__device__ __forceinline__ void gn_stats_pair(float v0, float v1, float q0, float q1, int n, int n_end, int cpg, float* cta_stats, int lane)
{
#pragma unroll
    for (int off = 4; off < 32; off <<= 1) {
        v0 += __shfl_xor_sync(0xffffffffu, v0, off); v1 += __shfl_xor_sync(0xffffffffu, v1, off);
        q0 += __shfl_xor_sync(0xffffffffu, q0, off); q1 += __shfl_xor_sync(0xffffffffu, q1, off);
    }
    if (lane < 4 && n < n_end) {
        const int g0 = n / cpg;
        if (n + 1 < n_end && (n + 1) / cpg == g0) { v0 += v1; q0 += q1; }
        else if (n + 1 < n_end) { atomicAdd(&cta_stats[2 * (g0 + 1)], v1); atomicAdd(&cta_stats[2 * (g0 + 1) + 1], q1); }
        atomicAdd(&cta_stats[2 * g0], v0);
        atomicAdd(&cta_stats[2 * g0 + 1], q0);
    }
}

__device__ __forceinline__ void gn_stats_flush(float* cta_stats, double* gstats, int groups, int t)
{
    if (t < 2 * groups) {
        const float v = atomicExch(&cta_stats[t], 0.f);
        if (v != 0.f) atomicAdd(&gstats[t], (double)v);
    }
}

}
```

Measured before the change: 164.0.

## Add multiple GEMM tile shapes chosen per problem by a wave-cost model

Templates the wgmma GEMM kernel on tile M/N (64 or 128 rows, 64 to 160 columns) and sizes the pipeline stage count to fit a fixed shared-memory ring. A cost model built from per-k-block timing constants, wave count and split-K reduction cost now picks the tile shape and split factor per GEMM/conv, instead of a fixed 128x128 tile with a heuristic split. The aim is to reduce wave quantization and tail under-utilisation on the many odd-sized SD UNet layers. In exchange it adds more kernel instantiations and relies on hard-coded cost constants that may mispredict.

```diff
diff --git a/include/onnxstream_b200_kernels.h b/include/onnxstream_b200_kernels.h
--- a/include/onnxstream_b200_kernels.h
+++ b/include/onnxstream_b200_kernels.h
@@ -138,6 +138,8 @@
 
 void osb_tc_set_pair_mode(int mode);
 
+void osb_tc_set_tile(int bm, int bn, int split);
+
 void osb_tc_profile(int enable);
 int osb_tc_profile_read(double* out4);
 int osb_tc_profile_dump(char* buf, int cap);
diff --git a/onnxstream_b200/csrc/gemm_wgmma.cu b/onnxstream_b200/csrc/gemm_wgmma.cu
--- a/onnxstream_b200/csrc/gemm_wgmma.cu
+++ b/onnxstream_b200/csrc/gemm_wgmma.cu
@@ -13,12 +13,23 @@
 constexpr int BLOCK_N = 128;
 constexpr int BLOCK_K = 64;
 constexpr int WG_K = 16;
-constexpr int STAGES = 6;
-constexpr int A_STAGE_BYTES = BLOCK_M * BLOCK_K * 2;
-constexpr int B_STAGE_BYTES = BLOCK_N * BLOCK_K * 2;
-constexpr int SMEM_BYTES = STAGES * (A_STAGE_BYTES + B_STAGE_BYTES) + 1024  + 256  + 2 * tcptx::GN_MAX_GROUPS * 4;
+constexpr int RING_BYTES = 6 * 32768;
 constexpr int NUM_THREADS = 384;
 constexpr int CONSUMER_THREADS = 256;
+
+template <int BM, int BN>
+struct TileCfg {
+    static constexpr int A_STAGE_BYTES = BM * BLOCK_K * 2;
+    static constexpr int B_STAGE_BYTES = BN * BLOCK_K * 2;
+    static constexpr int STAGES_FIT = RING_BYTES / (A_STAGE_BYTES + B_STAGE_BYTES);
+    static constexpr int STAGES = STAGES_FIT < 16 ? STAGES_FIT : 16;
+    static constexpr int WN = BM == 128 ? BN : BN / 2;
+    static constexpr int SMEM_BYTES = STAGES * (A_STAGE_BYTES + B_STAGE_BYTES) + 1024  + 256  + 2 * tcptx::GN_MAX_GROUPS * 4;
+    static_assert(BM == 64 || BM == 128, "BM");
+    static_assert(BN % 16 == 0 && B_STAGE_BYTES % 1024 == 0, "every stage and every warpgroup's B rows start on a 1024-byte swizzle boundary");
+};
+constexpr int A_STAGE_BYTES = TileCfg<BLOCK_M, BLOCK_N>::A_STAGE_BYTES;
+constexpr int B_STAGE_BYTES = TileCfg<BLOCK_M, BLOCK_N>::B_STAGE_BYTES;
 
 struct TcParams {
     int M, N, K;
@@ -45,30 +56,34 @@
     int f32_out;
     long long stride_c;
     long long ldc;
+    int bm, bn;
 };
 
 using namespace tcptx;
 
-template <int B_MN_MAJOR, bool BF16>
-__device__ __forceinline__ void mma_kblock(float (&acc)[64], uint64_t adesc, uint64_t bdesc)
+template <int WN, int B_MN_MAJOR, bool BF16>
+__device__ __forceinline__ void mma_kblock(float (&acc)[WN / 2], uint64_t adesc, uint64_t bdesc)
 {
     constexpr uint32_t b_kstep = B_MN_MAJOR ? (WG_K * 128) >> 4 : (WG_K * 2) >> 4;
     wgmma_fence();
 #pragma unroll
     for (int k = 0; k < BLOCK_K / WG_K; k++) {
         const uint64_t a = adesc + (uint64_t)(k * ((WG_K * 2) >> 4)), b = bdesc + (uint64_t)(k * b_kstep);
-        if (BF16) wgmma_m64n128k16_bf16<B_MN_MAJOR>(acc, a, b, 1u);
-        else wgmma_m64n128k16_f16<B_MN_MAJOR>(acc, a, b, 1u);
+        wgmma_ss<WN, B_MN_MAJOR, BF16>(acc, a, b, 1u);
     }
     wgmma_commit();
 }
 
 
-template <bool EXTRAS, int B_MN_MAJOR, bool BF16, bool PAIR>
+template <int BM, int BN, bool EXTRAS, int B_MN_MAJOR, bool BF16, bool PAIR>
 __global__ void __launch_bounds__(NUM_THREADS, 1)
 tc_gemm_kernel(const __grid_constant__ CUtensorMap map_a, const __grid_constant__ CUtensorMap map_b, const __grid_constant__ CUtensorMap map_b1,
                const __grid_constant__ CUtensorMap map_b2, const TcParams p)
 {
+    using Cfg = TileCfg<BM, BN>;
+    constexpr int STAGES = Cfg::STAGES, A_STAGE_BYTES = Cfg::A_STAGE_BYTES, B_STAGE_BYTES = Cfg::B_STAGE_BYTES, WN = Cfg::WN;
+    static_assert(!PAIR || (BM == 128 && BN == 128), "CTA pairs run 128 x 128 tiles");
+    static_assert(!B_MN_MAJOR || WN % 64 == 0, "an MN-major B is read in 64-column atoms");
     osb_pdl_trigger_entry();
     extern __shared__ uint8_t smem_raw[];
     uint8_t* smem = (uint8_t*)(((uintptr_t)smem_raw + 1023) & ~(uintptr_t)1023);
@@ -112,8 +127,8 @@
             int b = t2 / tiles_per_batch, r = t2 % tiles_per_batch;
             int mt = r % m_units, nt = r / m_units;
             if (PAIR) mt = 2 * mt + (int)rank;
-            int n0 = nt * BLOCK_N;
-            int y0 = 0, x0 = 0, m0 = mt * BLOCK_M;
+            int n0 = nt * BN;
+            int y0 = 0, x0 = 0, m0 = mt * BM;
             if (p.taps > 1 || p.bh > 0) { y0 = (mt / p.tiles_x) * p.bh; x0 = (mt % p.tiles_x) * p.bw; }
             const CUtensorMap* mbp = &map_b;
             if (p.groups > 1) { if (b == 1) mbp = &map_b1; else if (b == 2) mbp = &map_b2; b = 0; }
@@ -146,12 +161,10 @@
                         if (p.b_swap) tma_load_3d_s(sb, mbp, &full[stage], kglob, b, n0);
                         else tma_load_3d_s(sb, mbp, &full[stage], kglob, n0, b);
                     } else {
-                        if (p.b_swap) {
-                            tma_load_3d_s(sb, mbp, &full[stage], n0, b, kglob);
-                            tma_load_3d_s(sb + B_STAGE_BYTES / 2, mbp, &full[stage], n0 + 64, b, kglob);
-                        } else {
-                            tma_load_3d_s(sb, mbp, &full[stage], n0, kglob, b);
-                            tma_load_3d_s(sb + B_STAGE_BYTES / 2, mbp, &full[stage], n0 + 64, kglob, b);
+#pragma unroll
+                        for (int at = 0; at < BN / 64; at++) {
+                            if (p.b_swap) tma_load_3d_s(sb + at * 8192, mbp, &full[stage], n0 + 64 * at, b, kglob);
+                            else tma_load_3d_s(sb + at * 8192, mbp, &full[stage], n0 + 64 * at, kglob, b);
                         }
                     }
                 }
@@ -164,10 +177,11 @@
     } else if (warp >= 4) {
         const int wg = (warp >> 2) - 1;
         const int ct = (int)threadIdx.x - (NUM_THREADS - CONSUMER_THREADS);
-        const uint64_t adesc0 = make_smem_desc(smem_u32(smem_a) + wg * (BLOCK_M / 2) * 128, 16, 1024);
-        const uint64_t bdesc0 = p.b_kmajor ? make_smem_desc(smem_u32(smem_b), 16, 1024) : make_smem_desc(smem_u32(smem_b), B_STAGE_BYTES / 2, 1024);
+        const int wrow = BM == 128 ? 64 * wg : 0, wcol = BM == 128 ? 0 : WN * wg;
+        const uint64_t adesc0 = make_smem_desc(smem_u32(smem_a) + wrow * 128, 16, 1024);
+        const uint64_t bdesc0 = B_MN_MAJOR ? make_smem_desc(smem_u32(smem_b) + (wcol / 64) * 8192, 8192, 1024) : make_smem_desc(smem_u32(smem_b) + wcol * 128, 16, 1024);
         const bool partial = p.split_k > 1 || p.f32_out;
-        const int r_lo = wg * 64 + (warp & 3) * 16 + (lane >> 2);
+        const int r_lo = wrow + (warp & 3) * 16 + (lane >> 2);
         const int cq = 2 * (lane & 3);
         auto release = [&](int s) {
             if (PAIR) {
@@ -183,17 +197,17 @@
             int b = t2 / tiles_per_batch, r = t2 % tiles_per_batch;
             int mt = r % m_units, nt = r / m_units;
             if (PAIR) mt = 2 * mt + (int)rank;
-            const int n0 = nt * BLOCK_N;
-            const int n_end = min(p.N, n0 + BLOCK_N);
+            const int n0 = nt * BN, c0 = n0 + wcol;
+            const int n_end = min(p.N, n0 + BN);
             const int kb_lo = sp * kb_per_split, kb_hi = min(kb_lo + kb_per_split, k_blocks_all);
 
-            float acc[64];
+            float acc[WN / 2];
 #pragma unroll
-            for (int i = 0; i < 64; i++) acc[i] = 0.f;
+            for (int i = 0; i < WN / 2; i++) acc[i] = 0.f;
             int prev = -1;
             for (int kb = kb_lo; kb < kb_hi; kb++) {
                 mbar_wait(&full[stage], phase);
-                mma_kblock<B_MN_MAJOR, BF16>(acc, adesc0 + (uint64_t)(stage * (A_STAGE_BYTES >> 4)), bdesc0 + (uint64_t)(stage * (B_STAGE_BYTES >> 4)));
+                mma_kblock<WN, B_MN_MAJOR, BF16>(acc, adesc0 + (uint64_t)(stage * (A_STAGE_BYTES >> 4)), bdesc0 + (uint64_t)(stage * (B_STAGE_BYTES >> 4)));
                 if (prev >= 0) { wgmma_wait<1>(); release(prev); }
                 prev = stage;
                 if (++stage == STAGES) { stage = 0; phase ^= 1; }
@@ -211,7 +225,7 @@
                     row_ok[h] = y < p.Ho && x < p.Wo;
                     out_row[h] = (long long)y * p.Wo + x;
                 } else {
-                    int m = mt * BLOCK_M + row_in_tile;
+                    int m = mt * BM + row_in_tile;
                     row_ok[h] = m < p.M;
                     out_row[h] = m;
                 }
@@ -220,9 +234,9 @@
             if (p.groups > 1) cbase = b == 0 ? p.C : (b == 1 ? p.C1 : p.C2);
             const bool pair_ok = (p.N & 1) == 0 && (p.ldc & 1) == 0;
 #pragma unroll
-            for (int j = 0; j < BLOCK_N / 8; j++) {
-                if (n0 + 8 * j >= n_end) break;
-                const int n = n0 + 8 * j + cq;
+            for (int j = 0; j < WN / 8; j++) {
+                if (c0 + 8 * j >= n_end) break;
+                const int n = c0 + 8 * j + cq;
                 const bool ok0 = n < n_end, ok1 = n + 1 < n_end;
                 float s0 = 0.f, s1 = 0.f, q0 = 0.f, q1 = 0.f;
                 float add0 = 0.f, add1 = 0.f;
@@ -319,23 +333,108 @@
 
 int num_sms();
 
-int choose_split(int tiles, int k_blocks, size_t out_elems, cudaStream_t st, OsbWorkspace** ws_out)
-{
-    static const int forced = [] { const char* e = getenv("OSB_TC_SPLIT"); return e ? atoi(e) : 0; }();
-    *ws_out = nullptr;
-    static const int min_kb = [] { const char* e = getenv("OSB_TC_SPLIT_MINKB"); int v = e ? atoi(e) : 0; return v > 0 ? v : 32; }();
-    if ((tiles >= 100 && forced <= 0) || k_blocks < 4 || (k_blocks < min_kb && forced <= 0)) return 1;
-    int split = forced > 0 ? forced : num_sms() / tiles;
-    split = std::min(split, k_blocks / 2);
+int old_split(int tiles, int k_blocks, size_t out_elems)
+{
+    if (tiles >= 100 || k_blocks < 32) return 1;
+    int split = std::min(num_sms() / tiles, k_blocks / 2);
     while (split > 1 && (size_t)split * out_elems * 4 > WS_MAX) split--;
     if (split <= 1) return 1;
     int kb_per = (k_blocks + split - 1) / split;
-    split = (k_blocks + kb_per - 1) / kb_per;
+    return (k_blocks + kb_per - 1) / kb_per;
+}
+
+#define TC_TILES_KMAJOR(X) X(128, 128, 468.0) X(128, 64, 327.0) X(128, 80, 365.0) X(128, 160, 606.0) X(64, 64, 266.0) X(64, 128, 329.0) X(64, 160, 358.0)
+#define TC_TILES_MNMAJOR(X) X(128, 128, 499.0) X(128, 64, 284.0) X(64, 128, 300.0)
+struct TileShape { int bm, bn; double kb_ns; };
+#define TC_SHAPE(bm, bn, kb_ns) { bm, bn, kb_ns },
+const TileShape kTilesK[] = { TC_TILES_KMAJOR(TC_SHAPE) };
+const TileShape kTilesMN[] = { TC_TILES_MNMAJOR(TC_SHAPE) };
+#undef TC_SHAPE
+
+int g_tile_bm = 0, g_tile_bn = 0, g_tile_split = 0;
+
+struct TileProblem {
+    int M, N;
+    int Ho, Wo;
+    int conv, batch, k_blocks, kmajor;
+    bool may_split;
+    bool only_128;
+};
+struct TilePick { int bm, bn, split; };
+
+int conv_box_w(int bm, int Wo) { uint32_t r = 1; while ((int)r < Wo) r <<= 1; return std::min<int>(bm, (int)r); }
+int problem_m_tiles(const TileProblem& q, int bm)
+{
+    if (!q.conv) return (q.M + bm - 1) / bm;
+    const int bw = conv_box_w(bm, q.Wo), bh = bm / bw;
+    return ((q.Wo + bw - 1) / bw) * ((q.Ho + bh - 1) / bh);
+}
+
+constexpr double WAVE_NS = 4500.0;
+constexpr double REDUCE_NS = 4050.0;
+constexpr double REDUCE_NS_PER_BYTE = 2.6e-5;
+
+double tile_cost(const TileProblem& q, const TileShape& t, int split)
+{
+    const long long ctas = (long long)problem_m_tiles(q, t.bm) * ((q.N + t.bn - 1) / t.bn) * q.batch * split;
+    const long long waves = (ctas + num_sms() - 1) / num_sms();
+    const int kb_cta = (q.k_blocks + split - 1) / split;
+    const double reduce_bytes = (double)q.batch * q.M * q.N * (4.0 * split + 2.0);
+    return (double)waves * (kb_cta * t.kb_ns + WAVE_NS) + (split > 1 ? REDUCE_NS + REDUCE_NS_PER_BYTE * reduce_bytes : 0.0);
+}
+
+int split_for(const TileProblem& q, int tiles, int waves)
+{
+    if (!q.may_split || q.k_blocks < 4) return 1;
+    int split = std::min(waves * num_sms() / std::max(tiles, 1), q.k_blocks / 2);
+    while (split > 1 && (size_t)split * q.batch * q.M * q.N * 4 > WS_MAX) split--;
     if (split <= 1) return 1;
-    OsbWorkspace* ws = osb_workspace(st, OSB_WS_SPLITK);
-    if (!ws) return 1;
-    *ws_out = ws;
-    return split;
+    int kb_per = (q.k_blocks + split - 1) / split;
+    return (q.k_blocks + kb_per - 1) / kb_per;
+}
+
+TilePick choose_tile(const TileProblem& q)
+{
+    if (g_tile_bm < 0 || q.only_128) {
+        const int tiles = problem_m_tiles(q, BLOCK_M) * ((q.N + BLOCK_N - 1) / BLOCK_N) * q.batch;
+        return { BLOCK_M, BLOCK_N, q.may_split && q.k_blocks >= 4 ? old_split(tiles, q.k_blocks, (size_t)q.batch * q.M * q.N) : 1 };
+    }
+    const TileShape* shapes = q.kmajor ? kTilesK : kTilesMN;
+    const int n_shapes = q.kmajor ? (int)(sizeof(kTilesK) / sizeof(kTilesK[0])) : (int)(sizeof(kTilesMN) / sizeof(kTilesMN[0]));
+    bool forced_shape = false;
+    for (int i = 0; i < n_shapes; i++)
+        forced_shape |= (g_tile_bm > 0 || g_tile_bn > 0) && (g_tile_bm <= 0 || shapes[i].bm == g_tile_bm) && (g_tile_bn <= 0 || shapes[i].bn == g_tile_bn);
+    const bool forced_split = g_tile_split > 0 && (forced_shape || (g_tile_bm <= 0 && g_tile_bn <= 0));
+    TilePick best{ BLOCK_M, BLOCK_N, 1 };
+    double best_t = 1e300;
+    for (int i = 0; i < n_shapes; i++) {
+        const int bm = shapes[i].bm, bn = shapes[i].bn;
+        if (forced_shape && ((g_tile_bm > 0 && bm != g_tile_bm) || (g_tile_bn > 0 && bn != g_tile_bn))) continue;
+        const int tiles = problem_m_tiles(q, bm) * ((q.N + bn - 1) / bn) * q.batch;
+        int cand[3] = { 1, split_for(q, tiles, 1), split_for(q, tiles, 2) };
+        if (forced_split) {
+            int sp = q.may_split && q.k_blocks >= 2 ? std::min(g_tile_split, q.k_blocks) : 1;
+            while (sp > 1 && (size_t)sp * q.batch * q.M * q.N * 4 > WS_MAX) sp--;
+            if (sp > 1) { int kb_per = (q.k_blocks + sp - 1) / sp; sp = (q.k_blocks + kb_per - 1) / kb_per; }
+            cand[0] = cand[1] = cand[2] = std::max(sp, 1);
+        }
+        for (int sp : cand) {
+            const double t = tile_cost(q, shapes[i], sp);
+            if (t < best_t) { best_t = t; best = { bm, bn, sp }; }
+        }
+    }
+    return best;
+}
+
+TilePick choose_tile_ws(TileProblem q, cudaStream_t st, OsbWorkspace** ws_out)
+{
+    *ws_out = nullptr;
+    TilePick t = choose_tile(q);
+    if (t.split > 1) {
+        *ws_out = osb_workspace(st, OSB_WS_SPLITK);
+        if (!*ws_out) { q.may_split = false; t = choose_tile(q); }
+    }
+    return t;
 }
 
 bool make_map_rb(CUtensorMap* map, const void* base, uint64_t inner, uint64_t rows, uint64_t batch, uint64_t row_stride_bytes, uint64_t batch_stride_bytes,
@@ -356,7 +455,7 @@
     return n;
 }
 
-struct ProfRec { cudaEvent_t a, b; double flops, bytes; int M, N, K, taps, batch, split, conv; };
+struct ProfRec { cudaEvent_t a, b; double flops, bytes; int M, N, K, taps, batch, split, conv, bm, bn, kmajor; };
 bool g_prof = false;
 std::vector<ProfRec> g_prof_list;
 
@@ -369,47 +468,61 @@
     double a_bytes = (p.bh > 0 ? M * (p.K / kdiv) : M * Kt) * es * B;
     rec.bytes = a_bytes + N * Kt * es * (p.bh > 0 ? 1.0 : B) + M * N * es * B * (p.residual ? 2.0 : 1.0) + (p.bias ? N * es : 0.0);
     rec.M = p.M; rec.N = p.N; rec.K = p.K; rec.taps = p.taps; rec.batch = p.batch; rec.split = p.split_k; rec.conv = p.bh > 0;
+    rec.bm = p.bm; rec.bn = p.bn; rec.kmajor = p.b_kmajor;
     cudaEventRecord(rec.a, st);
 }
 
 using TcKernel = void (*)(CUtensorMap, CUtensorMap, CUtensorMap, CUtensorMap, TcParams);
+
+template <int BM, int BN, bool EXTRAS, int B_MN_MAJOR, bool BF16, bool PAIR>
+TcKernel ready_kernel(int* err)
+{
+    static const cudaError_t e = cudaFuncSetAttribute(tc_gemm_kernel<BM, BN, EXTRAS, B_MN_MAJOR, BF16, PAIR>, cudaFuncAttributeMaxDynamicSharedMemorySize,
+                                                      TileCfg<BM, BN>::SMEM_BYTES);
+    *err = (int)e;
+    return tc_gemm_kernel<BM, BN, EXTRAS, B_MN_MAJOR, BF16, PAIR>;
+}
+
+TcKernel pick_kernel(const TcParams& p, bool extras, bool pair, int* smem, int* err)
+{
+    *err = 0;
+    *smem = TileCfg<BLOCK_M, BLOCK_N>::SMEM_BYTES;
+    if (pair) {
+        if (p.bf16 || p.split_k != 1 || p.groups > 1 || p.bm != 128 || p.bn != 128) return nullptr;
+        return extras ? (p.b_kmajor ? ready_kernel<128, 128, true, 0, false, true>(err) : ready_kernel<128, 128, true, 1, false, true>(err))
+                      : (p.b_kmajor ? ready_kernel<128, 128, false, 0, false, true>(err) : ready_kernel<128, 128, false, 1, false, true>(err));
+    }
+    if (p.bf16) {
+        if (p.bm != 128 || p.bn != 128) return nullptr;
+        return p.b_kmajor ? ready_kernel<128, 128, false, 0, true, false>(err) : ready_kernel<128, 128, false, 1, true, false>(err);
+    }
+#define TC_PICK_K(M_, N_, COST_) \
+    if (p.bm == M_ && p.bn == N_) { *smem = TileCfg<M_, N_>::SMEM_BYTES; return extras ? ready_kernel<M_, N_, true, 0, false, false>(err) : ready_kernel<M_, N_, false, 0, false, false>(err); }
+#define TC_PICK_MN(M_, N_, COST_) \
+    if (p.bm == M_ && p.bn == N_) { *smem = TileCfg<M_, N_>::SMEM_BYTES; return ready_kernel<M_, N_, false, 1, false, false>(err); }
+    if (p.b_kmajor) { TC_TILES_KMAJOR(TC_PICK_K) }
+    else if (!extras) { TC_TILES_MNMAJOR(TC_PICK_MN) }
+#undef TC_PICK_K
+#undef TC_PICK_MN
+    return nullptr;
+}
 
 int launch(const CUtensorMap& ma, const CUtensorMap& mb, const TcParams& p, cudaStream_t st, const CUtensorMap* mb1p = nullptr, const CUtensorMap* mb2p = nullptr,
            bool pair = false)
 {
     const CUtensorMap& mb1 = mb1p ? *mb1p : mb;
     const CUtensorMap& mb2 = mb2p ? *mb2p : mb;
-    static bool attr_set = false;
-    if (!attr_set) {
-        TcKernel kernels[] = {
-            tc_gemm_kernel<false, 0, false, false>, tc_gemm_kernel<false, 1, false, false>, tc_gemm_kernel<true, 0, false, false>, tc_gemm_kernel<true, 1, false, false>,
-            tc_gemm_kernel<false, 0, true, false>, tc_gemm_kernel<false, 1, true, false>,
-            tc_gemm_kernel<false, 0, false, true>, tc_gemm_kernel<false, 1, false, true>, tc_gemm_kernel<true, 0, false, true>, tc_gemm_kernel<true, 1, false, true> };
-        for (auto k : kernels) {
-            cudaError_t e = cudaFuncSetAttribute(k, cudaFuncAttributeMaxDynamicSharedMemorySize, SMEM_BYTES);
-            if (e != cudaSuccess) return (int)e;
-        }
-        attr_set = true;
-    }
     const bool extras = p.bias2 != nullptr || p.gn_stats != nullptr;
-    TcKernel k;
-    if (pair) {
-        if (p.bf16 || p.split_k != 1 || p.groups > 1) return (int)cudaErrorInvalidValue;
-        k = extras ? (p.b_kmajor ? tc_gemm_kernel<true, 0, false, true> : tc_gemm_kernel<true, 1, false, true>)
-                   : (p.b_kmajor ? tc_gemm_kernel<false, 0, false, true> : tc_gemm_kernel<false, 1, false, true>);
-    } else if (p.bf16) {
-        k = p.b_kmajor ? tc_gemm_kernel<false, 0, true, false> : tc_gemm_kernel<false, 1, true, false>;
-    } else if (extras) {
-        k = p.b_kmajor ? tc_gemm_kernel<true, 0, false, false> : tc_gemm_kernel<true, 1, false, false>;
-    } else {
-        k = p.b_kmajor ? tc_gemm_kernel<false, 0, false, false> : tc_gemm_kernel<false, 1, false, false>;
-    }
+    int smem = 0, err = 0;
+    TcKernel k = pick_kernel(p, extras, pair, &smem, &err);
+    if (err) return err;
+    if (!k) return (int)cudaErrorInvalidValue;
     int grid;
     if (pair) {
         static int max_clusters = 0;
         if (!max_clusters) {
             cudaLaunchConfig_t cfg{};
-            cfg.gridDim = dim3(2 * (num_sms() / 2)); cfg.blockDim = dim3(NUM_THREADS); cfg.dynamicSmemBytes = SMEM_BYTES;
+            cfg.gridDim = dim3(2 * (num_sms() / 2)); cfg.blockDim = dim3(NUM_THREADS); cfg.dynamicSmemBytes = smem;
             cudaLaunchAttribute attr[1];
             attr[0].id = cudaLaunchAttributeClusterDimension;
             attr[0].val.clusterDim.x = 2; attr[0].val.clusterDim.y = 1; attr[0].val.clusterDim.z = 1;
@@ -425,7 +538,7 @@
     }
     ProfRec rec{};
     if (g_prof) prof_begin(rec, p, st);
-    osb_launch_cluster(k, grid, NUM_THREADS, (size_t)SMEM_BYTES, st, pair ? 2u : 1u, ma, mb, mb1, mb2, p);
+    osb_launch_cluster(k, grid, NUM_THREADS, (size_t)smem, st, pair ? 2u : 1u, ma, mb, mb1, mb2, p);
     if (p.f32_out) {
         launched(1);
         const long long total = (long long)p.batch * p.M * p.N;
@@ -471,6 +584,11 @@
 
 extern "C" void osb_tc_set_pair_mode(int mode) { g_pair_mode = mode; }
 
+extern "C" void osb_tc_set_tile(int bm, int bn, int split)
+{
+    g_tile_bm = bm; g_tile_bn = bm < 0 ? 0 : bn; g_tile_split = bm < 0 ? 0 : split;
+}
+
 extern "C" void osb_tc_profile(int enable)
 {
     for (auto& r : g_prof_list) { cudaEventDestroy(r.a); cudaEventDestroy(r.b); }
@@ -497,7 +615,8 @@
     for (auto& r : g_prof_list) {
         float t = 0.f;
         if (cudaEventSynchronize(r.b) != cudaSuccess || cudaEventElapsedTime(&t, r.a, r.b) != cudaSuccess) return -1;
-        int n = snprintf(buf + off, cap - off, "%d %d %d %d %d %d %d %.4f %.3f\n", r.M, r.N, r.K, r.taps, r.batch, r.split, r.conv, t, r.flops * 1e-9);
+        int n = snprintf(buf + off, cap - off, "%d %d %d %d %d %d %d %.4f %.3f %d %d %d\n", r.M, r.N, r.K, r.taps, r.batch, r.split, r.conv, t, r.flops * 1e-9,
+                         r.bm, r.bn, r.kmajor);
         if (n < 0 || off + n >= cap) break;
         off += n;
     }
@@ -651,26 +770,29 @@
         }
         return 0;
     }
+    const int64_t k_blocks = (K + BLOCK_K - 1) / BLOCK_K;
+    const bool pair = !g_f32x && use_pair((M + BLOCK_M - 1) / BLOCK_M, N);
+    const bool split_ok = ldc == N && (sc == M * N || batch == 1) && ((uintptr_t)residual & 7) == 0;
+    TileProblem q{ (int)M, (int)N, 0, 0, 0, (int)batch, (int)k_blocks, bt ? 1 : 0, split_ok && !pair, g_f32x != 0 };
+    OsbWorkspace* wsp = nullptr;
+    const TilePick t = pair ? TilePick{ BLOCK_M, BLOCK_N, 1 } : choose_tile_ws(q, st, &wsp);
     int a_swap = 0, b_swap = 0;
-    if (!make_map_rb(&ma, A, (uint64_t)K, (uint64_t)M, abatch, (uint64_t)lda * 2, (uint64_t)(sa ? sa : M * lda) * 2, BLOCK_K, BLOCK_M, &a_swap)) return (int)cudaErrorInvalidValue;
-    int64_t m_tiles = (M + BLOCK_M - 1) / BLOCK_M;
-    const bool pair = !g_f32x && use_pair(m_tiles, N);
-    bool okb = bt ? make_map_rb(&mb, B, (uint64_t)K, (uint64_t)N, bbatch, (uint64_t)ldb * 2, (uint64_t)(sb ? sb : N * ldb) * 2, BLOCK_K, pair ? BLOCK_N / 2 : BLOCK_N, &b_swap)
+    if (!make_map_rb(&ma, A, (uint64_t)K, (uint64_t)M, abatch, (uint64_t)lda * 2, (uint64_t)(sa ? sa : M * lda) * 2, BLOCK_K, t.bm, &a_swap)) return (int)cudaErrorInvalidValue;
+    bool okb = bt ? make_map_rb(&mb, B, (uint64_t)K, (uint64_t)N, bbatch, (uint64_t)ldb * 2, (uint64_t)(sb ? sb : N * ldb) * 2, BLOCK_K, pair ? BLOCK_N / 2 : t.bn, &b_swap)
                   : make_map_rb(&mb, B, (uint64_t)N, (uint64_t)K, bbatch, (uint64_t)ldb * 2, (uint64_t)(sb ? sb : K * ldb) * 2, 64, BLOCK_K, &b_swap);
     if (!okb) return (int)cudaErrorInvalidValue;
     TcParams p{};
     p.M = (int)M; p.N = (int)N; p.K = (int)K; p.batch = (int)batch;
-    p.m_tiles = (int)m_tiles; p.n_tiles = (int)((N + BLOCK_N - 1) / BLOCK_N);
+    p.bm = t.bm; p.bn = t.bn;
+    p.m_tiles = (int)((M + t.bm - 1) / t.bm); p.n_tiles = (int)((N + t.bn - 1) / t.bn);
     p.b_kmajor = bt ? 1 : 0;
     p.a_swap = a_swap; p.b_swap = b_swap;
     p.taps = 1; p.kw = 1; p.bh = 0; p.bw = 0; p.tiles_x = 1;
-    p.k_blocks_per_tap = (int)((K + BLOCK_K - 1) / BLOCK_K);
+    p.k_blocks_per_tap = (int)k_blocks;
     p.stride = 1;
     p.C = (__half*)C; p.bias = (const __half*)bias; p.residual = (const __half*)residual; p.stride_c = sc; p.ldc = ldc;
-    if (pair) { p.split_k = 1; return launch(ma, mb, p, st, nullptr, nullptr, true); }
-    OsbWorkspace* wsp = nullptr;
-    const bool split_ok = ldc == N && (sc == M * N || batch == 1) && ((uintptr_t)residual & 7) == 0;
-    p.split_k = split_ok ? choose_split(p.m_tiles * p.n_tiles * p.batch, p.k_blocks_per_tap, (size_t)batch * M * N, st, &wsp) : 1;
+    p.split_k = t.split;
+    if (pair) return launch(ma, mb, p, st, nullptr, nullptr, true);
     p.ws = wsp ? wsp->splitk : nullptr;
     if (g_f32x && !f32x_params(p, wsp, st)) return (int)cudaErrorNotSupported;
     return launch(ma, mb, p, st);
@@ -680,20 +802,21 @@
                                int64_t lda, int64_t ldb, int64_t ldc)
 {
     if (groups < 2 || groups > 3) return (int)cudaErrorInvalidValue;
+    const TilePick t = choose_tile(TileProblem{ (int)M, (int)N, 0, 0, 0, groups, (int)((K + BLOCK_K - 1) / BLOCK_K), bt ? 1 : 0, false, false });
     CUtensorMap ma, mb[3];
     int a_swap = 0, b_swap = 0;
-    if (!make_map_rb(&ma, A, (uint64_t)K, (uint64_t)M, 1, (uint64_t)lda * 2, (uint64_t)(M * lda) * 2, BLOCK_K, BLOCK_M, &a_swap)) return (int)cudaErrorInvalidValue;
-    int64_t m_tiles = (M + BLOCK_M - 1) / BLOCK_M;
+    if (!make_map_rb(&ma, A, (uint64_t)K, (uint64_t)M, 1, (uint64_t)lda * 2, (uint64_t)(M * lda) * 2, BLOCK_K, t.bm, &a_swap)) return (int)cudaErrorInvalidValue;
     for (int g = 0; g < groups; g++) {
         int sw = 0;
-        bool ok = bt ? make_map_rb(&mb[g], B[g], (uint64_t)K, (uint64_t)N, 1, (uint64_t)ldb * 2, (uint64_t)(N * ldb) * 2, BLOCK_K, BLOCK_N, &sw)
+        bool ok = bt ? make_map_rb(&mb[g], B[g], (uint64_t)K, (uint64_t)N, 1, (uint64_t)ldb * 2, (uint64_t)(N * ldb) * 2, BLOCK_K, t.bn, &sw)
                      : make_map_rb(&mb[g], B[g], (uint64_t)N, (uint64_t)K, 1, (uint64_t)ldb * 2, (uint64_t)(K * ldb) * 2, 64, BLOCK_K, &sw);
         if (!ok || (g > 0 && sw != b_swap)) return (int)cudaErrorInvalidValue;
         b_swap = sw;
     }
     TcParams p{};
     p.M = (int)M; p.N = (int)N; p.K = (int)K; p.batch = groups; p.groups = groups;
-    p.m_tiles = (int)m_tiles; p.n_tiles = (int)((N + BLOCK_N - 1) / BLOCK_N);
+    p.bm = t.bm; p.bn = t.bn;
+    p.m_tiles = (int)((M + t.bm - 1) / t.bm); p.n_tiles = (int)((N + t.bn - 1) / t.bn);
     p.b_kmajor = bt ? 1 : 0;
     p.a_swap = a_swap; p.b_swap = b_swap;
     p.taps = 1; p.kw = 1; p.bh = 0; p.bw = 0; p.tiles_x = 1;
@@ -722,39 +845,37 @@
     if (gn_done) *gn_done = 0;
     if (gn_stats && (gn_groups < 1 || gn_groups > tcptx::GN_MAX_GROUPS || Cout % gn_groups || Cout % 8)) gn_stats = nullptr;
     const int gn_cpg = gn_stats ? (int)(Cout / gn_groups) : 0;
-    uint32_t bw = std::min<uint32_t>(128, next_pow2((uint32_t)Wo)), bh = 128 / bw;
+    const int k_blocks = kh * kw * (int)((Cin + BLOCK_K - 1) / BLOCK_K);
+    TileProblem q{ (int)(Ho * Wo), (int)Cout, (int)Ho, (int)Wo, 1, 1, k_blocks, 1, false, g_f32x != 0 };
+    const bool pair = !g_f32x && Cout % 8 == 0 && use_pair(problem_m_tiles(q, BLOCK_M), Cout);
+    q.may_split = !pair && Cout % 4 == 0 && ((uintptr_t)residual & 7) == 0;
+    OsbWorkspace* wsp = nullptr;
+    const TilePick t = pair ? TilePick{ BLOCK_M, BLOCK_N, 1 } : choose_tile_ws(q, st, &wsp);
+    const uint32_t bw = (uint32_t)conv_box_w(t.bm, (int)Wo), bh = (uint32_t)t.bm / bw;
     CUtensorMap ma, mb;
     if (!make_map(&ma, x, (uint64_t)Cin, (uint64_t)W, (uint64_t)H, (uint64_t)Cin * 2, (uint64_t)W * Cin * 2, BLOCK_K, bw * stride, bh * stride, (uint32_t)stride))
         return (int)cudaErrorInvalidValue;
     int64_t Ktot = (int64_t)kh * kw * Cin;
-    const int64_t m_tiles_ = ((Wo + bw - 1) / bw) * ((Ho + bh - 1) / bh);
-    const bool pair = !g_f32x && Cout % 8 == 0 && use_pair(m_tiles_, Cout);
-    if (!make_map(&mb, w, (uint64_t)Ktot, (uint64_t)Cout, 1, (uint64_t)Ktot * 2, (uint64_t)Ktot * Cout * 2, BLOCK_K, pair ? BLOCK_N / 2 : BLOCK_N, 1))
+    if (!make_map(&mb, w, (uint64_t)Ktot, (uint64_t)Cout, 1, (uint64_t)Ktot * 2, (uint64_t)Ktot * Cout * 2, BLOCK_K, pair ? BLOCK_N / 2 : t.bn, 1))
         return (int)cudaErrorInvalidValue;
     TcParams p{};
     p.M = (int)(Ho * Wo); p.N = (int)Cout; p.K = (int)Cin; p.batch = 1;
+    p.bm = t.bm; p.bn = t.bn;
     p.tiles_x = (int)((Wo + bw - 1) / bw);
     p.m_tiles = p.tiles_x * (int)((Ho + bh - 1) / bh);
-    p.n_tiles = (int)((Cout + BLOCK_N - 1) / BLOCK_N);
+    p.n_tiles = (int)((Cout + t.bn - 1) / t.bn);
     p.b_kmajor = 1;
     p.taps = kh * kw; p.kw = kw; p.pad_top = pad_top; p.pad_left = pad_left; p.Wo = (int)Wo; p.Ho = (int)Ho; p.bw = (int)bw; p.bh = (int)bh;
     p.k_blocks_per_tap = (int)((Cin + BLOCK_K - 1) / BLOCK_K);
     p.stride = stride;
     p.C = (__half*)y; p.bias = (const __half*)bias; p.residual = (const __half*)residual; p.stride_c = 0; p.ldc = Cout;
-    if (pair) {
-        p.split_k = 1;
-        p.bias2 = (const __half*)bias2;
-        if (gn_stats) { p.gn_stats = gn_stats; p.gn_cpg = gn_cpg; p.gn_groups = gn_groups; if (gn_done) *gn_done = 1; }
-        { static const int dbg = env_int("OSB_GN_DEBUG"); p.gn_debug = dbg; }
-        return launch(ma, mb, p, st, nullptr, nullptr, true);
-    }
-    OsbWorkspace* wsp = nullptr;
-    p.split_k = (Cout % 4 == 0 && ((uintptr_t)residual & 7) == 0) ? choose_split(p.m_tiles * p.n_tiles, p.taps * p.k_blocks_per_tap, (size_t)Ho * Wo * Cout, st, &wsp) : 1;
+    p.split_k = t.split;
     p.ws = wsp ? wsp->splitk : nullptr;
     p.bias2 = (const __half*)bias2;
     const bool stats_ok = gn_stats && (p.split_k == 1 || gn_cpg % 4 == 0);
     if (stats_ok) { p.gn_stats = gn_stats; p.gn_cpg = gn_cpg; p.gn_groups = gn_groups; if (gn_done) *gn_done = 1; }
     { static const int dbg = env_int("OSB_GN_DEBUG"); p.gn_debug = dbg; }
+    if (pair) return launch(ma, mb, p, st, nullptr, nullptr, true);
     if (g_f32x) {
         if (!f32x_params(p, wsp, st)) return (int)cudaErrorNotSupported;
     }
diff --git a/onnxstream_b200/csrc/tc_ptx.cuh b/onnxstream_b200/csrc/tc_ptx.cuh
--- a/onnxstream_b200/csrc/tc_ptx.cuh
+++ b/onnxstream_b200/csrc/tc_ptx.cuh
@@ -144,65 +144,42 @@
 template <int N>
 __device__ __forceinline__ void wgmma_wait() { asm volatile("wgmma.wait_group.sync.aligned %0;" ::"n"(N) : "memory"); }
 
-template <int TRANS_B>
-__device__ __forceinline__ void wgmma_m64n128k16_f16(float (&d)[64], uint64_t da, uint64_t db, uint32_t scale_d)
-{
-    asm volatile(
-        "{\n\t.reg .pred p;\n\tsetp.ne.b32 p, %66, 0;\n\t"
-        "wgmma.mma_async.sync.aligned.m64n128k16.f32.f16.f16 "
-        "{%0, %1, %2, %3, %4, %5, %6, %7, %8, %9, %10, %11, %12, %13, %14, %15, %16, %17, %18, %19, %20, %21, %22, %23, %24, %25, %26, %27, %28, %29, %30, %31, %32, %33, %34, %35, %36, %37, %38, %39, %40, %41, %42, %43, %44, %45, %46, %47, %48, %49, %50, %51, %52, %53, %54, %55, %56, %57, %58, %59, %60, %61, %62, %63}, %64, %65, p, 1, 1, 0, %67;\n\t}"
-        : "+f"(d[0]), "+f"(d[1]), "+f"(d[2]), "+f"(d[3]), "+f"(d[4]), "+f"(d[5]), "+f"(d[6]), "+f"(d[7]), "+f"(d[8]), "+f"(d[9]), "+f"(d[10]), "+f"(d[11]), "+f"(d[12]), "+f"(d[13]), "+f"(d[14]), "+f"(d[15]), "+f"(d[16]), "+f"(d[17]), "+f"(d[18]), "+f"(d[19]), "+f"(d[20]), "+f"(d[21]), "+f"(d[22]), "+f"(d[23]), "+f"(d[24]), "+f"(d[25]), "+f"(d[26]), "+f"(d[27]), "+f"(d[28]), "+f"(d[29]), "+f"(d[30]), "+f"(d[31]), "+f"(d[32]), "+f"(d[33]), "+f"(d[34]), "+f"(d[35]), "+f"(d[36]), "+f"(d[37]), "+f"(d[38]), "+f"(d[39]), "+f"(d[40]), "+f"(d[41]), "+f"(d[42]), "+f"(d[43]), "+f"(d[44]), "+f"(d[45]), "+f"(d[46]), "+f"(d[47]), "+f"(d[48]), "+f"(d[49]), "+f"(d[50]), "+f"(d[51]), "+f"(d[52]), "+f"(d[53]), "+f"(d[54]), "+f"(d[55]), "+f"(d[56]), "+f"(d[57]), "+f"(d[58]), "+f"(d[59]), "+f"(d[60]), "+f"(d[61]), "+f"(d[62]), "+f"(d[63])
-        : "l"(da), "l"(db), "r"(scale_d), "n"(TRANS_B));
-}
-template <int TRANS_B>
-__device__ __forceinline__ void wgmma_m64n64k16_f16(float (&d)[32], uint64_t da, uint64_t db, uint32_t scale_d)
-{
-    asm volatile(
-        "{\n\t.reg .pred p;\n\tsetp.ne.b32 p, %34, 0;\n\t"
-        "wgmma.mma_async.sync.aligned.m64n64k16.f32.f16.f16 "
-        "{%0, %1, %2, %3, %4, %5, %6, %7, %8, %9, %10, %11, %12, %13, %14, %15, %16, %17, %18, %19, %20, %21, %22, %23, %24, %25, %26, %27, %28, %29, %30, %31}, %32, %33, p, 1, 1, 0, %35;\n\t}"
-        : "+f"(d[0]), "+f"(d[1]), "+f"(d[2]), "+f"(d[3]), "+f"(d[4]), "+f"(d[5]), "+f"(d[6]), "+f"(d[7]), "+f"(d[8]), "+f"(d[9]), "+f"(d[10]), "+f"(d[11]), "+f"(d[12]), "+f"(d[13]), "+f"(d[14]), "+f"(d[15]), "+f"(d[16]), "+f"(d[17]), "+f"(d[18]), "+f"(d[19]), "+f"(d[20]), "+f"(d[21]), "+f"(d[22]), "+f"(d[23]), "+f"(d[24]), "+f"(d[25]), "+f"(d[26]), "+f"(d[27]), "+f"(d[28]), "+f"(d[29]), "+f"(d[30]), "+f"(d[31])
-        : "l"(da), "l"(db), "r"(scale_d), "n"(TRANS_B));
-}
-template <int TRANS_B>
-__device__ __forceinline__ void wgmma_m64n32k16_f16(float (&d)[16], uint64_t da, uint64_t db, uint32_t scale_d)
-{
-    asm volatile(
-        "{\n\t.reg .pred p;\n\tsetp.ne.b32 p, %18, 0;\n\t"
-        "wgmma.mma_async.sync.aligned.m64n32k16.f32.f16.f16 "
-        "{%0, %1, %2, %3, %4, %5, %6, %7, %8, %9, %10, %11, %12, %13, %14, %15}, %16, %17, p, 1, 1, 0, %19;\n\t}"
-        : "+f"(d[0]), "+f"(d[1]), "+f"(d[2]), "+f"(d[3]), "+f"(d[4]), "+f"(d[5]), "+f"(d[6]), "+f"(d[7]), "+f"(d[8]), "+f"(d[9]), "+f"(d[10]), "+f"(d[11]), "+f"(d[12]), "+f"(d[13]), "+f"(d[14]), "+f"(d[15])
-        : "l"(da), "l"(db), "r"(scale_d), "n"(TRANS_B));
-}
-template <int TRANS_B>
-__device__ __forceinline__ void wgmma_m64n128k16_bf16(float (&d)[64], uint64_t da, uint64_t db, uint32_t scale_d)
-{
-    asm volatile(
-        "{\n\t.reg .pred p;\n\tsetp.ne.b32 p, %66, 0;\n\t"
-        "wgmma.mma_async.sync.aligned.m64n128k16.f32.bf16.bf16 "
-        "{%0, %1, %2, %3, %4, %5, %6, %7, %8, %9, %10, %11, %12, %13, %14, %15, %16, %17, %18, %19, %20, %21, %22, %23, %24, %25, %26, %27, %28, %29, %30, %31, %32, %33, %34, %35, %36, %37, %38, %39, %40, %41, %42, %43, %44, %45, %46, %47, %48, %49, %50, %51, %52, %53, %54, %55, %56, %57, %58, %59, %60, %61, %62, %63}, %64, %65, p, 1, 1, 0, %67;\n\t}"
-        : "+f"(d[0]), "+f"(d[1]), "+f"(d[2]), "+f"(d[3]), "+f"(d[4]), "+f"(d[5]), "+f"(d[6]), "+f"(d[7]), "+f"(d[8]), "+f"(d[9]), "+f"(d[10]), "+f"(d[11]), "+f"(d[12]), "+f"(d[13]), "+f"(d[14]), "+f"(d[15]), "+f"(d[16]), "+f"(d[17]), "+f"(d[18]), "+f"(d[19]), "+f"(d[20]), "+f"(d[21]), "+f"(d[22]), "+f"(d[23]), "+f"(d[24]), "+f"(d[25]), "+f"(d[26]), "+f"(d[27]), "+f"(d[28]), "+f"(d[29]), "+f"(d[30]), "+f"(d[31]), "+f"(d[32]), "+f"(d[33]), "+f"(d[34]), "+f"(d[35]), "+f"(d[36]), "+f"(d[37]), "+f"(d[38]), "+f"(d[39]), "+f"(d[40]), "+f"(d[41]), "+f"(d[42]), "+f"(d[43]), "+f"(d[44]), "+f"(d[45]), "+f"(d[46]), "+f"(d[47]), "+f"(d[48]), "+f"(d[49]), "+f"(d[50]), "+f"(d[51]), "+f"(d[52]), "+f"(d[53]), "+f"(d[54]), "+f"(d[55]), "+f"(d[56]), "+f"(d[57]), "+f"(d[58]), "+f"(d[59]), "+f"(d[60]), "+f"(d[61]), "+f"(d[62]), "+f"(d[63])
-        : "l"(da), "l"(db), "r"(scale_d), "n"(TRANS_B));
-}
-template <int TRANS_B>
-__device__ __forceinline__ void wgmma_m64n64k16_bf16(float (&d)[32], uint64_t da, uint64_t db, uint32_t scale_d)
-{
-    asm volatile(
-        "{\n\t.reg .pred p;\n\tsetp.ne.b32 p, %34, 0;\n\t"
-        "wgmma.mma_async.sync.aligned.m64n64k16.f32.bf16.bf16 "
-        "{%0, %1, %2, %3, %4, %5, %6, %7, %8, %9, %10, %11, %12, %13, %14, %15, %16, %17, %18, %19, %20, %21, %22, %23, %24, %25, %26, %27, %28, %29, %30, %31}, %32, %33, p, 1, 1, 0, %35;\n\t}"
-        : "+f"(d[0]), "+f"(d[1]), "+f"(d[2]), "+f"(d[3]), "+f"(d[4]), "+f"(d[5]), "+f"(d[6]), "+f"(d[7]), "+f"(d[8]), "+f"(d[9]), "+f"(d[10]), "+f"(d[11]), "+f"(d[12]), "+f"(d[13]), "+f"(d[14]), "+f"(d[15]), "+f"(d[16]), "+f"(d[17]), "+f"(d[18]), "+f"(d[19]), "+f"(d[20]), "+f"(d[21]), "+f"(d[22]), "+f"(d[23]), "+f"(d[24]), "+f"(d[25]), "+f"(d[26]), "+f"(d[27]), "+f"(d[28]), "+f"(d[29]), "+f"(d[30]), "+f"(d[31])
-        : "l"(da), "l"(db), "r"(scale_d), "n"(TRANS_B));
-}
-template <int TRANS_B>
-__device__ __forceinline__ void wgmma_m64n32k16_bf16(float (&d)[16], uint64_t da, uint64_t db, uint32_t scale_d)
-{
-    asm volatile(
-        "{\n\t.reg .pred p;\n\tsetp.ne.b32 p, %18, 0;\n\t"
-        "wgmma.mma_async.sync.aligned.m64n32k16.f32.bf16.bf16 "
-        "{%0, %1, %2, %3, %4, %5, %6, %7, %8, %9, %10, %11, %12, %13, %14, %15}, %16, %17, p, 1, 1, 0, %19;\n\t}"
-        : "+f"(d[0]), "+f"(d[1]), "+f"(d[2]), "+f"(d[3]), "+f"(d[4]), "+f"(d[5]), "+f"(d[6]), "+f"(d[7]), "+f"(d[8]), "+f"(d[9]), "+f"(d[10]), "+f"(d[11]), "+f"(d[12]), "+f"(d[13]), "+f"(d[14]), "+f"(d[15])
-        : "l"(da), "l"(db), "r"(scale_d), "n"(TRANS_B));
+#define TC_R8(a, b, c, d, e, f, g, h) "%" #a ", %" #b ", %" #c ", %" #d ", %" #e ", %" #f ", %" #g ", %" #h
+#define TC_R16 TC_R8(0, 1, 2, 3, 4, 5, 6, 7) ", " TC_R8(8, 9, 10, 11, 12, 13, 14, 15)
+#define TC_R32 TC_R16 ", " TC_R8(16, 17, 18, 19, 20, 21, 22, 23) ", " TC_R8(24, 25, 26, 27, 28, 29, 30, 31)
+#define TC_R40 TC_R32 ", " TC_R8(32, 33, 34, 35, 36, 37, 38, 39)
+#define TC_R64 TC_R40 ", " TC_R8(40, 41, 42, 43, 44, 45, 46, 47) ", " TC_R8(48, 49, 50, 51, 52, 53, 54, 55) ", " TC_R8(56, 57, 58, 59, 60, 61, 62, 63)
+#define TC_R80 TC_R64 ", " TC_R8(64, 65, 66, 67, 68, 69, 70, 71) ", " TC_R8(72, 73, 74, 75, 76, 77, 78, 79)
+#define TC_D8(i) "+f"(d[i]), "+f"(d[i + 1]), "+f"(d[i + 2]), "+f"(d[i + 3]), "+f"(d[i + 4]), "+f"(d[i + 5]), "+f"(d[i + 6]), "+f"(d[i + 7])
+#define TC_D16 TC_D8(0), TC_D8(8)
+#define TC_D32 TC_D16, TC_D8(16), TC_D8(24)
+#define TC_D40 TC_D32, TC_D8(32)
+#define TC_D64 TC_D40, TC_D8(40), TC_D8(48), TC_D8(56)
+#define TC_D80 TC_D64, TC_D8(64), TC_D8(72)
+#define TC_WGMMA_SS(N, TY, NAME, R, ODA, ODB, OSC, OTB, ...)                                                                                 \
+    template <int TRANS_B>                                                                                                              \
+    __device__ __forceinline__ void NAME(float (&d)[N / 2], uint64_t da, uint64_t db, uint32_t scale_d)                                 \
+    {                                                                                                                                   \
+        asm volatile("{\n\t.reg .pred p;\n\tsetp.ne.b32 p, " OSC ", 0;\n\t"                                                              \
+                     "wgmma.mma_async.sync.aligned.m64n" #N "k16.f32." TY "." TY " {" R "}, " ODA ", " ODB ", p, 1, 1, 0, " OTB ";\n\t}" \
+                     : __VA_ARGS__ : "l"(da), "l"(db), "r"(scale_d), "n"(TRANS_B));                                                     \
+    }
+#define TC_WGMMA_SS2(N, R, ODA, ODB, OSC, OTB, ...)                                      \
+    TC_WGMMA_SS(N, "f16", wgmma_m64n##N##k16_f16, R, ODA, ODB, OSC, OTB, __VA_ARGS__)   \
+    TC_WGMMA_SS(N, "bf16", wgmma_m64n##N##k16_bf16, R, ODA, ODB, OSC, OTB, __VA_ARGS__)
+TC_WGMMA_SS2(32, TC_R16, "%16", "%17", "%18", "%19", TC_D16)
+TC_WGMMA_SS2(64, TC_R32, "%32", "%33", "%34", "%35", TC_D32)
+TC_WGMMA_SS2(80, TC_R40, "%40", "%41", "%42", "%43", TC_D40)
+TC_WGMMA_SS2(128, TC_R64, "%64", "%65", "%66", "%67", TC_D64)
+TC_WGMMA_SS2(160, TC_R80, "%80", "%81", "%82", "%83", TC_D80)
+
+template <int N, int TRANS_B, bool BF16>
+__device__ __forceinline__ void wgmma_ss(float (&d)[N / 2], uint64_t da, uint64_t db, uint32_t scale_d)
+{
+#define TC_CASE(n) if constexpr (N == n) { if constexpr (BF16) wgmma_m64n##n##k16_bf16<TRANS_B>(d, da, db, scale_d); else wgmma_m64n##n##k16_f16<TRANS_B>(d, da, db, scale_d); }
+    TC_CASE(32) TC_CASE(64) TC_CASE(80) TC_CASE(128) TC_CASE(160)
+#undef TC_CASE
+    static_assert(N == 32 || N == 64 || N == 80 || N == 128 || N == 160, "no wgmma wrapper for this N");
 }
 __device__ __forceinline__ void wgmma_m64n128k32_u8(int32_t (&d)[64], uint64_t da, uint64_t db, uint32_t scale_d)
 {
```

Result: faster. 184.6 (median of 6 runs) (+12.5%).
